# aliftffd/ViT-vs-Raw-IQ

Hardware: AMD Instinct MI355X
Metric: IQ frames/sec training (fwd+loss+bwd+clip+AdamW) (higher is better)
Workload: dtype bf16; 1 GPU; ViT-Tiny/16 224x224 C=1 19cls (BASELINE configs[1]); config_id=B, per_gpu_batch=256, global_batch=256, parallelism=dp1, hipgraph=True

## Files before the change

### include/iqvit.h

```cpp
#ifndef IQVIT_H
#define IQVIT_H
#include <stddef.h>
#include <stdint.h>

#ifdef __cplusplus
extern "C" {
#endif

typedef void* iq_stream_t;

enum { IQ_STATUS_OK = 0, IQ_STATUS_ARG = 1, IQ_STATUS_UNSUPPORTED = 2, IQ_STATUS_LAUNCH = 3 };

typedef struct iq_dropout {
  uint64_t seed;
  uint32_t step;
  uint32_t site;
  float p;
  const uint32_t* step_dev;
} iq_dropout_t;
#define IQ_SITE_IMPAIR 0xFFFFFFFFu
#define IQ_SITE_SYNTH 0xFFFFFFFEu

int iq_ln_supported(int D);
int iq_ln_fwd(const void* z, const float* gamma, const float* beta, void* x, float* mean, float* rstd, int M, int D,
              float eps, iq_stream_t stream);
size_t iq_ln_bwd_ws_bytes(int D);
int iq_ln_bwd(const void* dx, const void* z, const float* mean, const float* rstd, const float* gamma, void* dz,
              void* dy, const iq_dropout_t* drop, float* dgamma, float* dbeta, float* ws, int accumulate, int M,
              int D, iq_stream_t stream);
int iq_ln_bwd_partial_rows(int M, int D);

typedef struct iq_epilogue {
  const float* bias;
  int relu;
  const float* pe;
  int tok, seq, cls_off;
  iq_dropout_t drop;
  const void* gate;
  int ldg;
  float gate_scale;
  const void* residual;
  int ldr;
} iq_epilogue_t;
int iq_gemm_bf16_nt(const void* A, int lda, const void* B, int ldb, void* C, int ldc, int M, int N, int K,
                    const iq_epilogue_t* epi, iq_stream_t stream);

int iq_gemm_ln_supported(int D, int K);
int iq_gemm_bf16_ln(const void* A, int lda, const void* W, int ldw, const float* bias, const void* residual, int ldr,
                    const iq_dropout_t* drop, const float* gamma, const float* beta, float eps, void* Z, void* X,
                    float* mean, float* rstd, int M, int D, int K, iq_stream_t stream);
// ... 25 lines not shown
                              const iq_dropout_t* drop2, const float* gamma2, const float* beta2, float eps, void* Z2, void* X,
                              float* mean2, float* rstd2, void* gate_bits, const void* Wq, const float* bq, void* Yq, int frames,
                              int S, int D, int F, iq_stream_t stream);

size_t iq_wgrad_ws_bytes(int M, int N, int K);
int iq_gemm_bf16_wgrad(const void* dY, int ldy, const void* X, int ldx, float* dW, float* dbias, int M, int N, int K,
                       float* ws, size_t ws_bytes, int accumulate, iq_stream_t stream);

typedef struct iq_wgrad_problem {
  const void* dY;
  int ldy;
  const void* X;
  int ldx;
  float* dW;
  float* dbias;
  int N, K;
} iq_wgrad_problem_t;
typedef struct iq_reduce_seg {
  const float* partials;
  int rows;
  int64_t row_stride;
  float* out;
  int64_t n;
} iq_reduce_seg_t;
size_t iq_wgrad_grouped_ws_bytes(const iq_wgrad_problem_t* probs, int nprob, int M, int max_workgroups);
int iq_gemm_bf16_wgrad_grouped(const iq_wgrad_problem_t* probs, int nprob, int M, float* ws, size_t ws_bytes,
                               int accumulate, int max_workgroups, const iq_reduce_seg_t* extra, int nextra,
                               iq_stream_t stream);

int iq_attn_supported(int S, int dh);
int iq_attn_fwd(const void* qkv, void* out, float* lse, int B, int S, int H, int dh, iq_stream_t stream);
int iq_attn_bwd(const void* qkv, const void* out, const void* dout, const float* lse, void* dqkv, int B, int S, int H,
                int dh, iq_stream_t stream);
int iq_attn_fwd_masked(const void* qkv, void* out, float* lse, const uint8_t* mask, long mask_hstride, int B, int S,
                       int H, int dh, iq_stream_t stream);
int iq_attn_bwd_masked(const void* qkv, const void* out, const void* dout, const float* lse, void* dqkv,
                       const uint8_t* mask, long mask_hstride, int B, int S, int H, int dh, iq_stream_t stream);
int iq_attn_probs(const void* qkv, const float* lse, float* out, long out_bstride, int B, int S, int H, int dh,
                  int rows, int heads, iq_stream_t stream);
int iq_attn_grad_probs(const void* qkv, const float* lse, const void* dout, float* out, long out_bstride, int B, int S,
                       int H, int dh, int rows, int heads, int positive, iq_stream_t stream);
int iq_attn_relevance_step(const void* qkv, const float* lse, const void* dout, const float* r_in, float* r_out, int B,
                           int S, int H, int dh, iq_stream_t stream);

int iq_frames_preprocess(const float* raw, float* out, int n_frames, int len, int take, const float* stats,
                         iq_stream_t stream);
typedef struct iq_impair {
  float phase_lo, phase_hi;
  float cfo_lo, cfo_hi;
  int   rot90;
  int   conj;
  int   shift_max;
  float gain_db_lo, gain_db_hi;
  float snr_db_lo, snr_db_hi;
  uint64_t seed; uint32_t step;
  uint64_t frame_base;
} iq_impair_t;
int iq_frames_impair(const float* raw, float* out, float* drawn, int n_frames, int len, int take, const float* stats,
                     const iq_impair_t* imp, iq_stream_t stream);
#define IQ_SYNTH_MAX_CLASSES 128
#define IQ_SYNTH_MAX_SNRS 64
typedef struct iq_synth_class { int kind; int offset; int count; } iq_synth_class_t;
typedef struct iq_synth {
  const float* points;
  const iq_synth_class_t* classes; int n_classes;
  const float* snrs_db; int n_snrs;
// ... 26 lines not shown
size_t iq_gradnorm_ws_bytes(size_t n);
int iq_gradnorm_sq(const float* g, size_t n, float grad_scale, float* ws, float* out, iq_stream_t stream);
int iq_adamw_step(float* p, const float* g, float* m, float* v, void* shadow_bf16, size_t n, float lr, float beta1,
                  float beta2, float eps, float weight_decay, int step, const float* gnorm_sq, float max_norm,
                  float grad_scale, const float* dyn, iq_stream_t stream);
int iq_counter_add(uint32_t* ctr_u32, uint32_t inc_u32, float* ctr_f32, float inc_f32, iq_stream_t stream);
int iq_cast_bf16(const float* src, void* dst, size_t n, iq_stream_t stream);
int iq_transpose_cast_bf16(const float* src, void* dst, int rows, int cols, iq_stream_t stream);

typedef struct iq_model_cfg {
  int kind;
  int in_channels;
  int img_h, img_w, patch;
  int seq_length, conv_k, use_cls;
  int num_classes, d_model, n_head, n_layers, ffn_hidden;
  float drop_prob;
} iq_model_cfg_t;

typedef struct iq_model iq_model_t;

int iq_model_create(const iq_model_cfg_t* cfg, iq_model_t** out);
void iq_model_destroy(iq_model_t* m);
const char* iq_model_last_error(const iq_model_t* m);
int iq_model_tokens(const iq_model_t* m);
size_t iq_model_param_floats(const iq_model_t* m);
int iq_model_param_entries(const iq_model_t* m);
int iq_model_param_entry(const iq_model_t* m, int i, char* name, int name_cap, size_t* offset, int* ndim, int* dims);
size_t iq_model_shadow_bytes(const iq_model_t* m);
size_t iq_model_workspace_bytes(const iq_model_t* m, int batch, int training);
int iq_model_bind(iq_model_t* m, float* params, float* grads, const float* pe, void* shadow);
int iq_model_bind_step_counter(iq_model_t* m, uint32_t* counter);
int iq_model_refresh_shadow(iq_model_t* m, iq_stream_t stream);
int iq_model_refresh_transposed(iq_model_t* m, iq_stream_t stream);
int iq_model_forward(iq_model_t* m, const float* src, int batch, void* workspace, size_t ws_bytes, int training,
                     uint64_t seed, uint32_t step, float* enc_out, float* logits, iq_stream_t stream);
int iq_model_backward(iq_model_t* m, const float* dlogits, const float* denc, int batch, void* workspace,
                      size_t ws_bytes, int accumulate, int stage_hi, int stage_lo, iq_stream_t stream);
int iq_model_grad_range(const iq_model_t* m, int stage_hi, int stage_lo, size_t* off, size_t* len);
#define IQ_BWD_PARAM_GRADS 1
int iq_model_backward_input(iq_model_t* m, const float* dlogits, const float* denc, int batch, void* workspace,
                            size_t ws_bytes, float* dsrc, int flags, iq_stream_t stream);
int iq_model_attention(iq_model_t* m, const void* workspace, size_t ws_bytes, int batch, int layer, int rows,
                       int heads, float* out, long out_bstride, iq_stream_t stream);
int iq_model_attention_rollout(iq_model_t* m, const void* workspace, size_t ws_bytes, int batch, float alpha,
                               float* out, iq_stream_t stream);
int iq_model_attention_relevance(iq_model_t* m, const float* dlogits, int batch, void* workspace, size_t ws_bytes,
                                 float* rel, float* const* maps, int rows, int heads, int positive, long out_bstride,
                                 iq_stream_t stream);

#define IQ_PROF_FAMILIES 8
int iq_prof_enable(int on);
int iq_prof_collect(double* ms, long long* count);
size_t iq_prof_kernels(char* out, size_t cap, int reset);

#ifdef __cplusplus
}
#endif
#endif
```

### vit-vs-raw-iq_amd/_native.py

```python
from __future__ import annotations

import ctypes as C
import os

_HERE = os.path.dirname(os.path.abspath(__file__))
LIB_PATH = os.environ.get("IQ_LIBIQVIT") or os.path.join(_HERE, "libiqvit.so")

BWD_PARAM_GRADS = 1

STATUS = {0: "ok", 1: "invalid argument", 2: "unsupported shape/configuration", 3: "HIP launch error"}


class IqError(RuntimeError):
    pass


class Dropout(C.Structure):
    _fields_ = [("seed", C.c_uint64), ("step", C.c_uint32), ("site", C.c_uint32), ("p", C.c_float),
                ("step_dev", C.c_void_p)]


class Impair(C.Structure):
    _fields_ = [("phase_lo", C.c_float), ("phase_hi", C.c_float), ("cfo_lo", C.c_float), ("cfo_hi", C.c_float),
                ("rot90", C.c_int), ("conj", C.c_int), ("shift_max", C.c_int), ("gain_db_lo", C.c_float),
                ("gain_db_hi", C.c_float), ("snr_db_lo", C.c_float), ("snr_db_hi", C.c_float), ("seed", C.c_uint64),
                ("step", C.c_uint32), ("frame_base", C.c_uint64)]


class SynthClass(C.Structure):
    _fields_ = [("kind", C.c_int), ("offset", C.c_int), ("count", C.c_int)]


class Synth(C.Structure):
    _fields_ = [("points", C.c_void_p), ("classes", C.POINTER(SynthClass)), ("n_classes", C.c_int),
                ("snrs_db", C.POINTER(C.c_float)), ("n_snrs", C.c_int), ("balanced", C.c_int), ("seed", C.c_uint64),
                ("stream", C.c_uint32), ("frame_base", C.c_uint64)]


class Epilogue(C.Structure):
    _fields_ = [("bias", C.c_void_p), ("relu", C.c_int), ("pe", C.c_void_p), ("tok", C.c_int), ("seq", C.c_int),
                ("cls_off", C.c_int), ("drop", Dropout), ("gate", C.c_void_p), ("ldg", C.c_int),
                ("gate_scale", C.c_float), ("residual", C.c_void_p), ("ldr", C.c_int)]


class WgradProblem(C.Structure):
    _fields_ = [("dY", C.c_void_p), ("ldy", C.c_int), ("X", C.c_void_p), ("ldx", C.c_int), ("dW", C.c_void_p),
                ("dbias", C.c_void_p), ("N", C.c_int), ("K", C.c_int)]


class ReduceSeg(C.Structure):
    _fields_ = [("partials", C.c_void_p), ("rows", C.c_int), ("row_stride", C.c_int64), ("out", C.c_void_p),
                ("n", C.c_int64)]
# ... 9 lines not shown
_P, _I, _Z, _F = C.c_void_p, C.c_int, C.c_size_t, C.c_float
_U64, _U32 = C.c_uint64, C.c_uint32

SIGNATURES = {
    "iq_ln_supported": (_I, [_I]),
    "iq_ln_fwd": (_I, [_P, _P, _P, _P, _P, _P, _I, _I, _F, _P]),
    "iq_ln_bwd_ws_bytes": (_Z, [_I]),
    "iq_ln_bwd_partial_rows": (_I, [_I, _I]),
    "iq_ln_bwd": (_I, [_P, _P, _P, _P, _P, _P, _P, C.POINTER(Dropout), _P, _P, _P, _I, _I, _I, _P]),
    "iq_gemm_bf16_nt": (_I, [_P, _I, _P, _I, _P, _I, _I, _I, _I, C.POINTER(Epilogue), _P]),
    "iq_gemm_ln_supported": (_I, [_I, _I]),
    "iq_gemm_bf16_ln": (_I, [_P, _I, _P, _I, _P, _P, _I, C.POINTER(Dropout), _P, _P, _F, _P, _P, _P, _P, _I, _I, _I, _P]),
    "iq_gemm_lnbwd_supported": (_I, [_I, _I]),
    "iq_gemm_lnbwd_partial_rows": (_I, [_I]),
    "iq_gemm_bf16_lnbwd": (_I, [_P, _I, _P, _I, _P, _I, _P, _P, _P, _P, C.POINTER(Dropout), _P, _P, _P, _I, _I, _I, _P]),
    "iq_ffn_chain_supported": (_I, [_I, _I, _I]),
    "iq_ffn_chain_bwd_partial_rows": (_I, [_I]),
    "iq_ffn_chain_bwd": (_I, [_P, _P, _P, _F, _P, _P, _P, _P, _P, _P, _P, C.POINTER(Dropout), _P, _P, _P, _P, _P, _I, _I, _I, _I, _P]),
    "iq_qkv_dgrad_ffn_chain_bwd": (_I, [_P, _P, _P, _P, _P, _P, _P, C.POINTER(Dropout), _P, _P, _P,
                                        _P, _P, _F, _P, _P, _P, _P, _P, _P, _P, C.POINTER(Dropout), _P, _P, _P, _P, _P, _I, _I, _I, _I, _P]),
    "iq_ffn_chain_gate_bytes": (_Z, [_I, _I]),
    "iq_ffn_chain_fwd": (_I, [_P, _P, _P, C.POINTER(Dropout), _P, _P, _P, C.POINTER(Dropout), _P, _P, _F, _P, _P, _P, _P, _P, _I, _I,
                              _I, _I, _P]),
    "iq_attn_out_ffn_chain_fwd": (_I, [_P, _P, _P, C.POINTER(Dropout), _P, _P, _P, _P, _P, _P, _P,
                                       _P, _P, C.POINTER(Dropout), _P, _P, _P, C.POINTER(Dropout), _P, _P, _F, _P, _P, _P, _P, _P,
                                       _P, _P, _P, _I, _I, _I, _I, _P]),
    "iq_wgrad_ws_bytes": (_Z, [_I, _I, _I]),
    "iq_gemm_bf16_wgrad": (_I, [_P, _I, _P, _I, _P, _P, _I, _I, _I, _P, _Z, _I, _P]),
    "iq_wgrad_grouped_ws_bytes": (_Z, [_P, _I, _I, _I]),
    "iq_gemm_bf16_wgrad_grouped": (_I, [_P, _I, _I, _P, _Z, _I, _I, _P, _I, _P]),
    "iq_attn_supported": (_I, [_I, _I]),
    "iq_attn_fwd": (_I, [_P, _P, _P, _I, _I, _I, _I, _P]),
    "iq_attn_bwd": (_I, [_P, _P, _P, _P, _P, _I, _I, _I, _I, _P]),
    "iq_attn_fwd_masked": (_I, [_P, _P, _P, _P, C.c_long, _I, _I, _I, _I, _P]),
    "iq_attn_bwd_masked": (_I, [_P, _P, _P, _P, _P, _P, C.c_long, _I, _I, _I, _I, _P]),
    "iq_attn_probs": (_I, [_P, _P, _P, C.c_long, _I, _I, _I, _I, _I, _I, _P]),
    "iq_attn_grad_probs": (_I, [_P, _P, _P, _P, C.c_long, _I, _I, _I, _I, _I, _I, _I, _P]),
    "iq_attn_relevance_step": (_I, [_P, _P, _P, _P, _P, _I, _I, _I, _I, _P]),
    "iq_frames_preprocess": (_I, [_P, _P, _I, _I, _I, C.POINTER(C.c_float), _P]),
    "iq_frames_impair": (_I, [_P, _P, _P, _I, _I, _I, C.POINTER(C.c_float), C.POINTER(Impair), _P]),
    "iq_frames_synth": (_I, [_P, _P, _P, _P, _P, _I, _I, C.POINTER(Synth), _P]),
    "iq_patchify": (_I, [_P, _P, _I, _I, _I, _I, _I, _I, _I, _P]),
    "iq_cls_rows": (_I, [_P, _P, _P, _I, _I, _I, C.POINTER(Dropout), _P]),
    "iq_embed_bwd_gather": (_I, [_P, _P, _P, _I, _I, _I, _I, _I, C.POINTER(Dropout), _I, _P]),
    "iq_embed_dgrad": (_I, [_P, _P, _I, _P, _I, _I, _I, _I, _I, _I, _I, _P]),
    "iq_linf_step": (_I, [_P, _P, _P, _F, _F, _F, _F, _Z, _P]),
    "iq_head_fwd": (_I, [_P, _P, _P, _P, _P, _P, _P, _P, _I, _I, _I, _I, _I, _P]),
    "iq_ce_fwd_bwd": (_I, [_P, _P, _I, _I, _F, _F, _P, _P, _P, _P]),
    "iq_head_bwd": (_I, [_P, _P, _P, _P, _P, _P, _P, _P, _P, _P, _P, _I, _I, _I, _I, _I, _I, _P]),
    "iq_gradnorm_ws_bytes": (_Z, [_Z]),
    "iq_gradnorm_sq": (_I, [_P, _Z, _F, _P, _P, _P]),
    "iq_adamw_step": (_I, [_P, _P, _P, _P, _P, _Z, _F, _F, _F, _F, _F, _I, _P, _F, _F, _P, _P]),
    "iq_counter_add": (_I, [_P, _U32, _P, _F, _P]),
    "iq_cast_bf16": (_I, [_P, _P, _Z, _P]),
    "iq_transpose_cast_bf16": (_I, [_P, _P, _I, _I, _P]),
    "iq_model_create": (_I, [C.POINTER(ModelCfg), C.POINTER(_P)]),
    "iq_model_destroy": (None, [_P]),
    "iq_model_last_error": (C.c_char_p, [_P]),
    "iq_model_tokens": (_I, [_P]),
    "iq_model_param_floats": (_Z, [_P]),
    "iq_model_param_entries": (_I, [_P]),
    "iq_model_param_entry": (_I, [_P, _I, C.c_char_p, _I, C.POINTER(_Z), C.POINTER(_I), C.POINTER(_I)]),
    "iq_model_shadow_bytes": (_Z, [_P]),
    "iq_model_workspace_bytes": (_Z, [_P, _I, _I]),
    "iq_model_bind": (_I, [_P, _P, _P, _P, _P]),
    "iq_model_bind_step_counter": (_I, [_P, _P]),
# ... 52 lines not shown
```

### vit-vs-raw-iq_amd/csrc/attention.hip

```cpp
#include <stdlib.h>

#include "common.h"
#include "iqvit.h"
#include "prof.h"

namespace {

constexpr int ATT_THREADS = 512;
constexpr int ATT_WAVES = ATT_THREADS / 64;
constexpr float LOG2E = 1.4426950408889634f;
constexpr float LN2 = 0.6931471805599453f;
constexpr float NEG_BIG = -1.0e30f;

__device__ __forceinline__ float fast_exp2(float x) { return __builtin_amdgcn_exp2f(x); }

template <int DH> struct AttCfg {
  static constexpr int LD = (DH == 16) ? 16 : DH + 16;
  static constexpr int KS = (DH + 31) / 32;
  static constexpr int DT = DH / 16;
  static constexpr int CPR = DH / 8;
};

typedef __attribute__((address_space(3))) s16x4 lds_s16x4;

// ... 50 lines not shown
#pragma unroll
    for (int j = 0; j < UN; ++j) {
      const int id = base + j * ATT_THREADS + tid;
      const int r = id / CPR, c = id % CPR;
      if (id < total) {
        const bool live = r_begin + r < S;
        *reinterpret_cast<bf16x8*>(imgA + r * LD + c * 8) = live ? va[j] : bf16x8{};
        *reinterpret_cast<bf16x8*>(imgB + r * LD + c * 8) = live ? vb[j] : bf16x8{};
      }
    }
  }
}

__device__ __forceinline__ bf16x8 pack_b(const f32x4& lo, const f32x4& hi) {
  bf16x8 v;
#pragma unroll
  for (int r = 0; r < 4; ++r) { v[r] = (bf16)lo[r]; v[4 + r] = (bf16)hi[r]; }
  return v;
}

__device__ __forceinline__ float group4_max(float v) {
  v = fmaxf(v, __shfl_xor(v, 16, 64));
  return fmaxf(v, __shfl_xor(v, 32, 64));
}
__device__ __forceinline__ float group4_sum(float v) {
  v += __shfl_xor(v, 16, 64);
  return v + __shfl_xor(v, 32, 64);
}

template <int DH, bool MASKED>
__global__ __launch_bounds__(ATT_THREADS) void attn_fwd_kernel(const bf16* __restrict__ qkv, bf16* __restrict__ out,
                                                               float* __restrict__ lse, const uint8_t* __restrict__ mask,
                                                               long mask_hstride, int S, int H, int kchunk,
                                                               float scale_log2, float masked_raw) {
  using C = AttCfg<DH>;
  extern __shared__ __attribute__((aligned(16))) unsigned char smem[];
  bf16* Ks = reinterpret_cast<bf16*>(smem);
  bf16* Vs = Ks + kchunk * C::LD;
  const int tid = threadIdx.x, lane = tid & 63, wave = tid >> 6, g = lane >> 4, c16 = lane & 15;
  const int b = blockIdx.x / H, h = blockIdx.x % H;
  const int D = H * DH;
  const long ldg = 3L * D;
  const bf16* qb = qkv + (long)b * S * ldg + h * DH;
  const bf16* kb_ = qb + D;
  const bf16* vb_ = qb + 2 * D;
  const uint8_t* mk = MASKED ? mask + (long)b * (mask_hstride ? (long)H * S * S : (long)S * S) + h * mask_hstride : nullptr;
  const int qtiles = (S + 31) / 32, npass = (qtiles + ATT_WAVES - 1) / ATT_WAVES, nstage = (S + kchunk - 1) / kchunk;

  if (nstage == 1) {
    stage_pair<DH, 4>(Ks, kb_, ldg, Vs, vb_, ldg, 0, min(kchunk, ((S + 31) / 32) * 32), S, tid);
    __syncthreads();
  }
  for (int pass = 0; pass < npass; ++pass) {
    const int qt = pass * ATT_WAVES + wave;
    const bool active = qt < qtiles;
    bf16x8 qf[2][C::KS];
    f32x4 o[2][C::DT];
    float m[2], lsum[2];
#pragma unroll
    for (int u = 0; u < 2; ++u) {
      m[u] = NEG_BIG; lsum[u] = 0.f;
#pragma unroll
      for (int s = 0; s < C::KS; ++s) qf[u][s] = row_frag_gmem<DH>(qb, ldg, qt * 32 + u * 16 + c16, active ? S : 0, s, lane);
#pragma unroll
      for (int dt = 0; dt < C::DT; ++dt) o[u][dt] = f32x4{0.f, 0.f, 0.f, 0.f};
    }
    for (int st = 0; st < nstage; ++st) {
      const int k0 = st * kchunk;
      const int krows = min(kchunk, ((S - k0 + 31) / 32) * 32);
      if (nstage > 1) {
        __syncthreads();
        stage_pair<DH, 2>(Ks, kb_, ldg, Vs, vb_, ldg, k0, krows, S, tid);
        __syncthreads();
      }
      if (active) {
        const bool u1 = qt * 32 + 16 < S;
        for (int kb = 0; kb < krows; kb += 32) {
          const bool k1 = k0 + kb + 16 < S;
          const bool kpad = k0 + kb + 32 > S;
          f32x4 sc[2][2];
// ... 65 lines not shown
            const bf16x8 vt = tr_frag(Vs, C::LD, kb, dt * 16, lane);
            o[0][dt] = __builtin_amdgcn_mfma_f32_16x16x32_bf16(vt, pb[0], o[0][dt], 0, 0, 0);
            if (u1) o[1][dt] = __builtin_amdgcn_mfma_f32_16x16x32_bf16(vt, pb[1], o[1][dt], 0, 0, 0);
          }
        }
      }
    }
    if (active) {
#pragma unroll
      for (int u = 0; u < 2; ++u) {
        const float l = group4_sum(lsum[u]);
        const float inv = 1.0f / l;
        const int q = qt * 32 + u * 16 + c16;
        if (q < S) {
#pragma unroll
          for (int dt = 0; dt < C::DT; ++dt) {
            bf16x4 w;
#pragma unroll
            for (int r = 0; r < 4; ++r) w[r] = (bf16)(o[u][dt][r] * inv);
            *reinterpret_cast<bf16x4*>(out + ((long)b * S + q) * D + h * DH + dt * 16 + 4 * g) = w;
          }
          if (g == 0) lse[((long)b * H + h) * S + q] = (m[u] + log2f(l)) * LN2;
        }
      }
    }
  }
}

template <int DH, bool MASKED>
__global__ __launch_bounds__(ATT_THREADS, 4) void attn_bwd_kernel(const bf16* __restrict__ qkv, const bf16* __restrict__ out,
                                                               const bf16* __restrict__ dout, const float* __restrict__ lse,
                                                               bf16* __restrict__ dqkv, const uint8_t* __restrict__ mask,
                                                               long mask_hstride, int S, int H, int spad, int chunk,
                                                               float scale, float masked_raw) {
  using C = AttCfg<DH>;
  extern __shared__ __attribute__((aligned(16))) unsigned char smem[];
  bf16* I0 = reinterpret_cast<bf16*>(smem);
  bf16* I1 = I0 + chunk * C::LD;
  float* lse_s = reinterpret_cast<float*>(I1 + chunk * C::LD);
  float* del_s = lse_s + spad;
  const int tid = threadIdx.x, lane = tid & 63, wave = tid >> 6, g = lane >> 4, c16 = lane & 15;
  const int b = blockIdx.x / H, h = blockIdx.x % H;
  const int D = H * DH;
  const long ldg = 3L * D;
  const bf16* qb = qkv + (long)b * S * ldg + h * DH;
  const bf16* kb_ = qb + D;
  const bf16* vb_ = qb + 2 * D;
  const bf16* ob = out + (long)b * S * D + h * DH;
  const bf16* dob = dout + (long)b * S * D + h * DH;
  bf16* dqb = dqkv + (long)b * S * ldg + h * DH;
  const uint8_t* mk = MASKED ? mask + (long)b * (mask_hstride ? (long)H * S * S : (long)S * S) + h * mask_hstride : nullptr;
  const float scale_log2 = scale * LOG2E;
  const int nblk = spad / 32;
  const int nchunk = (spad + chunk - 1) / chunk;
  const bool single = nchunk == 1;

  if (single) {
    stage_pair<DH, 4>(I0, qb, ldg, I1, dob, (long)D, 0, spad, S, tid);
    __syncthreads();
  }
  for (int q = tid; q < spad; q += ATT_THREADS) {
    float dl = 0.f, ls = 0.f;
    if (q < S) {
#pragma unroll
      for (int c = 0; c < C::CPR; ++c) {
        const bf16x8 a = single ? *reinterpret_cast<const bf16x8*>(I1 + q * C::LD + c * 8)
                                : *reinterpret_cast<const bf16x8*>(dob + (long)q * D + c * 8);
        const bf16x8 o8 = *reinterpret_cast<const bf16x8*>(ob + (long)q * D + c * 8);
#pragma unroll
        for (int e = 0; e < 8; ++e) dl += (float)a[e] * (float)o8[e];
      }
      ls = lse[((long)b * H + h) * S + q] * LOG2E;
    }
    del_s[q] = dl;
    lse_s[q] = ls;
  }
  __syncthreads();

  const int nunit = (S + 15) / 16;
  for (int ug = 0; ug * ATT_WAVES < nunit; ++ug) {
    const int unit = ug * ATT_WAVES + wave;
    const bool have = unit < nunit;
    bf16x8 kf[C::KS], vf[C::KS];
#pragma unroll
    for (int s = 0; s < C::KS; ++s) {
      kf[s] = row_frag_gmem<DH>(kb_, ldg, unit * 16 + c16, have ? S : 0, s, lane);
      vf[s] = row_frag_gmem<DH>(vb_, ldg, unit * 16 + c16, have ? S : 0, s, lane);
    }
    f32x4 dv[C::DT], dk[C::DT];
#pragma unroll
    for (int dt = 0; dt < C::DT; ++dt) { dv[dt] = f32x4{0.f, 0.f, 0.f, 0.f}; dk[dt] = f32x4{0.f, 0.f, 0.f, 0.f}; }
    const int key = unit * 16 + c16;
    const bool unit_partial = unit * 16 + 16 > S;
    for (int qc = 0; qc < nchunk; ++qc) {
      const int q0 = qc * chunk;
      const int rows = min(chunk, spad - q0);
      if (!single) {
        __syncthreads();
        stage_pair<DH, 2>(I0, qb, ldg, I1, dob, (long)D, q0, rows, S, tid);
        __syncthreads();
      }
      if (!have) continue;
      for (int ql = 0; ql < rows; ql += 32) {
        const bool u1 = q0 + ql + 16 < S;
        f32x4 p[2], ds[2];
#pragma unroll
        for (int u = 0; u < 2; ++u) {
          if (u == 1 && !u1) { p[1] = f32x4{0.f, 0.f, 0.f, 0.f}; ds[1] = f32x4{0.f, 0.f, 0.f, 0.f}; continue; }
          f32x4 sa = {0.f, 0.f, 0.f, 0.f}, dp = {0.f, 0.f, 0.f, 0.f};
#pragma unroll
          for (int s = 0; s < C::KS; ++s) {
            const bf16x8 qa = row_frag_lds<DH>(I0, ql + u * 16 + c16, s, lane);
            const bf16x8 da = row_frag_lds<DH>(I1, ql + u * 16 + c16, s, lane);
            sa = __builtin_amdgcn_mfma_f32_16x16x32_bf16(qa, kf[s], sa, 0, 0, 0);
            dp = __builtin_amdgcn_mfma_f32_16x16x32_bf16(da, vf[s], dp, 0, 0, 0);
          }
#pragma unroll
          for (int r = 0; r < 4; ++r) {
            const int q = q0 + ql + u * 16 + 4 * g + r;
            bool blocked = false;
            if (MASKED) blocked = q < S && key < S && !mk[(long)q * S + key];
            float pv = fast_exp2((blocked ? masked_raw : sa[r]) * scale_log2 - lse_s[q]);
            if (unit_partial) pv = key < S ? pv : 0.f;
            p[u][r] = pv;
            ds[u][r] = blocked ? 0.f : pv * (dp[r] - del_s[q]) * scale;
          }
        }
        const bf16x8 pB = pack_b(p[0], p[1]), dsB = pack_b(ds[0], ds[1]);
#pragma unroll
        for (int dt = 0; dt < C::DT; ++dt) {
          const bf16x8 doT = tr_frag(I1, C::LD, ql, dt * 16, lane);
          const bf16x8 qT = tr_frag(I0, C::LD, ql, dt * 16, lane);
// ... 6 lines not shown
#pragma unroll
      for (int dt = 0; dt < C::DT; ++dt) {
        bf16x4 wk, wv;
#pragma unroll
        for (int r = 0; r < 4; ++r) { wk[r] = (bf16)dk[dt][r]; wv[r] = (bf16)dv[dt][r]; }
        *reinterpret_cast<bf16x4*>(dqb + (long)key * ldg + D + dt * 16 + 4 * g) = wk;
        *reinterpret_cast<bf16x4*>(dqb + (long)key * ldg + 2 * D + dt * 16 + 4 * g) = wv;
      }
    }
  }

  bf16x8 qf[2][C::KS], dof[2][C::KS];
  if (single) {
#pragma unroll
    for (int u = 0; u < 2; ++u)
#pragma unroll
      for (int s = 0; s < C::KS; ++s) {
        const int q = min(wave, nblk - 1) * 32 + u * 16 + c16;
        qf[u][s] = row_frag_lds<DH>(I0, q, s, lane);
        dof[u][s] = row_frag_lds<DH>(I1, q, s, lane);
      }
  }
  for (int qg = 0; qg * ATT_WAVES < nblk; ++qg) {
    const int qblk = qg * ATT_WAVES + wave;
    const bool have = qblk < nblk;
    float lq[2], dl[2];
#pragma unroll
    for (int u = 0; u < 2; ++u) {
      const int q = min(qblk, nblk - 1) * 32 + u * 16 + c16;
      if (!single || qg != 0) {
#pragma unroll
        for (int s = 0; s < C::KS; ++s) {
          qf[u][s] = row_frag_gmem<DH>(qb, ldg, q, have ? S : 0, s, lane);
          dof[u][s] = row_frag_gmem<DH>(dob, (long)D, q, have ? S : 0, s, lane);
        }
      }
      lq[u] = lse_s[q];
      dl[u] = del_s[q];
    }
    f32x4 dq[C::DT][2];
#pragma unroll
    for (int dt = 0; dt < C::DT; ++dt)
#pragma unroll
      for (int u = 0; u < 2; ++u) dq[dt][u] = f32x4{0.f, 0.f, 0.f, 0.f};
    for (int kc = 0; kc < nchunk; ++kc) {
      const int k0 = kc * chunk;
      const int rows = min(chunk, spad - k0);
      if (!single || qg == 0) {
        __syncthreads();
        stage_pair<DH, 2>(I0, kb_, ldg, I1, vb_, ldg, k0, rows, S, tid);
        __syncthreads();
      }
      if (!have) continue;
      const bool u1 = qblk * 32 + 16 < S;
      for (int kl = 0; kl < rows; kl += 32) {
        const bool kblk_partial = k0 + kl + 32 > S;
        const bool k1 = k0 + kl + 16 < S;
        f32x4 ds[2][2];
#pragma unroll
        for (int kt = 0; kt < 2; ++kt) {
          if (kt == 1 && !k1) { ds[0][1] = f32x4{0.f, 0.f, 0.f, 0.f}; ds[1][1] = f32x4{0.f, 0.f, 0.f, 0.f}; continue; }
          bf16x8 ka[C::KS], va[C::KS];
#pragma unroll
          for (int s = 0; s < C::KS; ++s) {
            ka[s] = row_frag_lds<DH>(I0, kl + kt * 16 + c16, s, lane);
            va[s] = row_frag_lds<DH>(I1, kl + kt * 16 + c16, s, lane);
          }
// ... 17 lines not shown
              float pv = fast_exp2((blocked ? masked_raw : sa[r]) * scale_log2 - lq[u]);
              if (kblk_partial) pv = key < S ? pv : 0.f;
              ds[u][kt][r] = blocked ? 0.f : pv * (dp[r] - dl[u]) * scale;
            }
          }
        }
        bf16x8 dsB[2];
#pragma unroll
        for (int u = 0; u < 2; ++u) dsB[u] = pack_b(ds[u][0], ds[u][1]);
#pragma unroll
        for (int dt = 0; dt < C::DT; ++dt) {
          const bf16x8 kT = tr_frag(I0, C::LD, kl, dt * 16, lane);
          dq[dt][0] = __builtin_amdgcn_mfma_f32_16x16x32_bf16(kT, dsB[0], dq[dt][0], 0, 0, 0);
          if (u1) dq[dt][1] = __builtin_amdgcn_mfma_f32_16x16x32_bf16(kT, dsB[1], dq[dt][1], 0, 0, 0);
        }
      }
    }
    if (have) {
#pragma unroll
      for (int u = 0; u < 2; ++u) {
        const int q = qblk * 32 + u * 16 + c16;
        if (q < S) {
#pragma unroll
          for (int dt = 0; dt < C::DT; ++dt) {
            bf16x4 w;
#pragma unroll
            for (int r = 0; r < 4; ++r) w[r] = (bf16)dq[dt][u][r];
            *reinterpret_cast<bf16x4*>(dqb + (long)q * ldg + dt * 16 + 4 * g) = w;
          }
        }
      }
    }
  }
}

constexpr int ONCE_MAX_SPAD = 224;
constexpr int ONCE_LD = 64;

__device__ __forceinline__ int once_off(int row, int col) { return row * ONCE_LD + (col ^ (((row >> 1) & 3) << 4)); }

__device__ __forceinline__ bf16x8 once_tr_frag(const bf16* tile, int r0, int dt, int lane) {
  const int i16 = lane & 15, g = lane >> 4;
  const bf16* a = tile + once_off(r0 + 4 * g + (i16 >> 2), dt * 16 + 4 * (i16 & 3));
  s16x4 lo = __builtin_amdgcn_ds_read_tr16_b64_v4i16((lds_s16x4*)(a));
  s16x4 hi = __builtin_amdgcn_ds_read_tr16_b64_v4i16((lds_s16x4*)(a + 16 * ONCE_LD));
  s16x8 v = {lo[0], lo[1], lo[2], lo[3], hi[0], hi[1], hi[2], hi[3]};
  return __builtin_bit_cast(bf16x8, v);
}
__device__ __forceinline__ bf16x8 once_row_frag(const bf16* tile, int row, int s, int lane) {
  return *reinterpret_cast<const bf16x8*>(tile + once_off(row, s * 32 + 8 * (lane >> 4)));
}

template <int NT, int UN, int NIMG>
__device__ __forceinline__ void once_stage(bf16* const (&img)[NIMG], const bf16* const (&base)[NIMG],
                                           const long (&ldg)[NIMG], int spad, int S, int tid) {
  const int total = spad * 8;
  for (int b0 = 0; b0 < total; b0 += UN * NT) {
    bf16x8 v[NIMG][UN];
#pragma unroll
    for (int j = 0; j < UN; ++j) {
      const int id = min(b0 + j * NT + tid, total - 1);
      const int r = min(id >> 3, S - 1), c = id & 7;
#pragma unroll
      for (int i = 0; i < NIMG; ++i) v[i][j] = *reinterpret_cast<const bf16x8*>(base[i] + (long)r * ldg[i] + c * 8);
    }
#pragma unroll
    for (int j = 0; j < UN; ++j) {
      const int id = b0 + j * NT + tid;
      const int r = id >> 3, c = id & 7;
      if (id < total) {
        const bool live = r < S;
#pragma unroll
        for (int i = 0; i < NIMG; ++i) *reinterpret_cast<bf16x8*>(img[i] + once_off(r, c * 8)) = live ? v[i][j] : bf16x8{};
      }
    }
  }
}

template <int NT>
__global__ __launch_bounds__(NT, 4) void attn_bwd_once_kernel(const bf16* __restrict__ qkv, const bf16* __restrict__ out,
                                                              const bf16* __restrict__ dout, const float* __restrict__ lse,
                                                              bf16* __restrict__ dqkv, int S, int H, int spad, float scale) {
  constexpr int DH = 64, KS = 2, DT = 4, NW = NT / 64;
  extern __shared__ __attribute__((aligned(16))) unsigned char smem[];
  bf16* I0 = reinterpret_cast<bf16*>(smem);
  bf16* I1 = I0 + spad * ONCE_LD;
  float* lse_s = reinterpret_cast<float*>(I1 + spad * ONCE_LD);
  float* del_s = lse_s + spad;
  bf16* dSi = reinterpret_cast<bf16*>(del_s + spad);
  const int tid = threadIdx.x, lane = tid & 63, wave = tid >> 6, g = lane >> 4, c16 = lane & 15;
  const int b = blockIdx.x / H, h = blockIdx.x % H;
  const int D = H * DH;
  const long ldg = 3L * D;
  const bf16* qb = qkv + (long)b * S * ldg + h * DH;
  const bf16* kb_ = qb + D;
  const bf16* vb_ = qb + 2 * D;
  const bf16* ob = out + (long)b * S * D + h * DH;
  const bf16* dob = dout + (long)b * S * D + h * DH;
  bf16* dqb = dqkv + (long)b * S * ldg + h * DH;
  const float scale_log2 = scale * LOG2E;
  const int nunit = (S + 15) / 16;
  const int ldS = nunit * 16 + 8;

  {
    bf16* const img[2] = {I0, I1};
    const bf16* const src[2] = {qb, dob};
    const long lds_[2] = {ldg, (long)D};
    once_stage<NT, 2048 / NT, 2>(img, src, lds_, spad, S, tid);
  }
  __syncthreads();
  for (int q = tid; q < spad; q += NT) {
    float dl = 0.f, ls = 0.f;
    if (q < S) {
#pragma unroll
      for (int c = 0; c < 8; ++c) {
        const bf16x8 a = *reinterpret_cast<const bf16x8*>(I1 + once_off(q, c * 8));
        const bf16x8 o8 = *reinterpret_cast<const bf16x8*>(ob + (long)q * D + c * 8);
#pragma unroll
        for (int e = 0; e < 8; ++e) dl += (float)a[e] * (float)o8[e];
      }
      ls = lse[((long)b * H + h) * S + q] * LOG2E;
    }
    del_s[q] = dl;
    lse_s[q] = ls;
  }
  __syncthreads();

  for (int unit = wave; unit < nunit; unit += NW) {
    bf16x8 kf[KS], vf[KS];
#pragma unroll
    for (int s = 0; s < KS; ++s) {
      kf[s] = row_frag_gmem<DH>(kb_, ldg, unit * 16 + c16, S, s, lane);
      vf[s] = row_frag_gmem<DH>(vb_, ldg, unit * 16 + c16, S, s, lane);
    }
    f32x4 dv[DT], dk[DT];
#pragma unroll
    for (int dt = 0; dt < DT; ++dt) { dv[dt] = f32x4{0.f, 0.f, 0.f, 0.f}; dk[dt] = f32x4{0.f, 0.f, 0.f, 0.f}; }
    const int key = unit * 16 + c16;
    const bool unit_partial = unit * 16 + 16 > S;
    for (int ql = 0; ql < spad; ql += 32) {
      const bool u1 = ql + 16 < S;
      f32x4 p[2], ds[2];
#pragma unroll
      for (int u = 0; u < 2; ++u) {
        if (u == 1 && !u1) { p[1] = f32x4{0.f, 0.f, 0.f, 0.f}; ds[1] = f32x4{0.f, 0.f, 0.f, 0.f}; continue; }
        f32x4 sa = {0.f, 0.f, 0.f, 0.f}, dp = {0.f, 0.f, 0.f, 0.f};
#pragma unroll
        for (int s = 0; s < KS; ++s) {
          const bf16x8 qa = once_row_frag(I0, ql + u * 16 + c16, s, lane);
          const bf16x8 da = once_row_frag(I1, ql + u * 16 + c16, s, lane);
          sa = __builtin_amdgcn_mfma_f32_16x16x32_bf16(qa, kf[s], sa, 0, 0, 0);
          dp = __builtin_amdgcn_mfma_f32_16x16x32_bf16(da, vf[s], dp, 0, 0, 0);
        }
        const f32x4 lq4 = *reinterpret_cast<const f32x4*>(lse_s + ql + u * 16 + 4 * g);
        const f32x4 dl4 = *reinterpret_cast<const f32x4*>(del_s + ql + u * 16 + 4 * g);
#pragma unroll
        for (int r = 0; r < 4; ++r) {
          float pv = fast_exp2(sa[r] * scale_log2 - lq4[r]);
          if (unit_partial) pv = key < S ? pv : 0.f;
          p[u][r] = pv;
          ds[u][r] = pv * (dp[r] - dl4[r]) * scale;
        }
      }
      const bf16x8 pB = pack_b(p[0], p[1]), dsB = pack_b(ds[0], ds[1]);
      bf16* w = dSi + (ql + 4 * g) * ldS + key;
#pragma unroll
      for (int r = 0; r < 4; ++r) w[r * ldS] = dsB[r];
      if (u1) {
#pragma unroll
        for (int r = 0; r < 4; ++r) w[(16 + r) * ldS] = dsB[4 + r];
      }
#pragma unroll
      for (int dt = 0; dt < DT; ++dt) {
        const bf16x8 doT = once_tr_frag(I1, ql, dt, lane);
        const bf16x8 qT = once_tr_frag(I0, ql, dt, lane);
        dv[dt] = __builtin_amdgcn_mfma_f32_16x16x32_bf16(doT, pB, dv[dt], 0, 0, 0);
        dk[dt] = __builtin_amdgcn_mfma_f32_16x16x32_bf16(qT, dsB, dk[dt], 0, 0, 0);
      }
    }
    if (key < S) {
#pragma unroll
      for (int dt = 0; dt < DT; ++dt) {
        bf16x4 wk, wv;
#pragma unroll
        for (int r = 0; r < 4; ++r) { wk[r] = (bf16)dk[dt][r]; wv[r] = (bf16)dv[dt][r]; }
        *reinterpret_cast<bf16x4*>(dqb + (long)key * ldg + D + dt * 16 + 4 * g) = wk;
        *reinterpret_cast<bf16x4*>(dqb + (long)key * ldg + 2 * D + dt * 16 + 4 * g) = wv;
      }
    }
  }

  __syncthreads();
  {
    bf16* const img[1] = {I0};
    const bf16* const src[1] = {kb_};
    const long lds_[1] = {ldg};
    once_stage<NT, 2048 / NT, 1>(img, src, lds_, spad, S, tid);
  }
  __syncthreads();
  for (int half = wave; half < nunit; half += NW) {
    const int q = half * 16 + c16;
    const bf16* drow = dSi + q * ldS + 4 * g;
    f32x4 dq[DT];
#pragma unroll
    for (int dt = 0; dt < DT; ++dt) dq[dt] = f32x4{0.f, 0.f, 0.f, 0.f};
    for (int kl = 0; kl < spad; kl += 32) {
      const bool k1 = kl + 16 < S;
      const bf16x4 lo = *reinterpret_cast<const bf16x4*>(drow + kl);
      bf16x4 hi = {};
      if (k1) hi = *reinterpret_cast<const bf16x4*>(drow + kl + 16);
      const bf16x8 dsB = {lo[0], lo[1], lo[2], lo[3], hi[0], hi[1], hi[2], hi[3]};
#pragma unroll
      for (int dt = 0; dt < DT; ++dt) {
        const bf16x8 kT = once_tr_frag(I0, kl, dt, lane);
        dq[dt] = __builtin_amdgcn_mfma_f32_16x16x32_bf16(kT, dsB, dq[dt], 0, 0, 0);
      }
    }
    if (q < S) {
#pragma unroll
      for (int dt = 0; dt < DT; ++dt) {
        bf16x4 w;
#pragma unroll
        for (int r = 0; r < 4; ++r) w[r] = (bf16)dq[dt][r];
        *reinterpret_cast<bf16x4*>(dqb + (long)q * ldg + dt * 16 + 4 * g) = w;
      }
    }
  }
}

template <int DH>
__device__ __forceinline__ bf16x8 row_frag_img(const bf16* tile, int ld, int row, int s, int lane) {
  const int d0 = s * 32 + 8 * (lane >> 4);
  bf16x8 v = {};
  if (DH >= 32 || d0 < DH) v = *reinterpret_cast<const bf16x8*>(tile + row * ld + d0);
// ... 376 lines not shown
  return iq_launch_status();
}
template <int DH>
int launch_frame_bwd(const void* qkv, const void* out, const void* dout, const float* lse, void* dqkv, int B, int S, int H,
                     hipStream_t st) {
  const int spad = (S + 31) / 32 * 32;
  const size_t lds = frame_bwd_lds(S, H, DH);
  auto k = attn_frame_bwd_kernel<DH, (DH == 64 ? 2 : 3), (DH == 16 ? 4 : DH == 32 ? 3 : 2)>;
  if (lds > 48 * 1024) (void)hipFuncSetAttribute((const void*)k, hipFuncAttributeMaxDynamicSharedMemorySize, (int)lds);
  const int threads = 64 * (H < ATT_WAVES ? H : ATT_WAVES);
  k<<<B, threads, lds, st>>>((const bf16*)qkv, (const bf16*)out, (const bf16*)dout, lse, (bf16*)dqkv, S, H, spad,
                             1.0f / sqrtf((float)DH));
  return iq_launch_status();
}

constexpr size_t ATT_LDS_FWD_BUDGET = 72 * 1024;
constexpr size_t ATT_LDS_BWD_BUDGET = 76 * 1024;
constexpr int ATT_MAX_S = 4096;

template <int DH> int bwd_chunk_rows(int S) {
  const int spad = (S + 31) / 32 * 32;
  const long room = (long)ATT_LDS_BWD_BUDGET - (long)2 * spad * sizeof(float);
  int chunk = (int)(room / (2 * AttCfg<DH>::LD * 2)) / 32 * 32;
  if (chunk > spad) chunk = spad;
  return chunk;
}
template <int DH> size_t bwd_lds_bytes(int S) {
  const int spad = (S + 31) / 32 * 32;
  return (size_t)2 * bwd_chunk_rows<DH>(S) * AttCfg<DH>::LD * 2 + (size_t)2 * spad * sizeof(float);
}

template <int DH, bool MASKED>
int launch_fwd(const void* qkv, void* out, float* lse, const uint8_t* mask, long mask_hstride, int B, int S, int H,
               hipStream_t st) {
  const int spad = (S + 31) / 32 * 32;
  int kchunk = (int)(ATT_LDS_FWD_BUDGET / (2 * AttCfg<DH>::LD * 2)) / 32 * 32;
  if (kchunk > spad) kchunk = spad;
  const size_t lds = (size_t)2 * kchunk * AttCfg<DH>::LD * 2;
  const float scale_log2 = LOG2E / sqrtf((float)DH);
  if (lds > 48 * 1024)
    (void)hipFuncSetAttribute((const void*)attn_fwd_kernel<DH, MASKED>, hipFuncAttributeMaxDynamicSharedMemorySize, (int)lds);
  attn_fwd_kernel<DH, MASKED><<<B * H, ATT_THREADS, lds, st>>>((const bf16*)qkv, (bf16*)out, lse, mask, mask_hstride, S, H,
                                                               kchunk, scale_log2, -10000.0f * sqrtf((float)DH));
  return iq_launch_status();
}

template <int DH, bool MASKED>
int launch_bwd(const void* qkv, const void* out, const void* dout, const float* lse, void* dqkv, const uint8_t* mask,
               long mask_hstride, int B, int S, int H, hipStream_t st) {
  const int spad = (S + 31) / 32 * 32;
  const int chunk = bwd_chunk_rows<DH>(S);
  if (S > ATT_MAX_S || chunk < 32) return IQ_ERR_UNSUPPORTED;
  const size_t lds = bwd_lds_bytes<DH>(S);
  if (lds > 48 * 1024)
    (void)hipFuncSetAttribute((const void*)attn_bwd_kernel<DH, MASKED>, hipFuncAttributeMaxDynamicSharedMemorySize, (int)lds);
  attn_bwd_kernel<DH, MASKED><<<B * H, ATT_THREADS, lds, st>>>((const bf16*)qkv, (const bf16*)out, (const bf16*)dout, lse,
                                                               (bf16*)dqkv, mask, mask_hstride, S, H, spad, chunk,
                                                               1.0f / sqrtf((float)DH), -10000.0f * sqrtf((float)DH));
  return iq_launch_status();
}

inline int once_threads(int S, int dh, bool masked) {
  static const int tune = [] { const char* e = getenv("IQ_TUNE_ATTN_BWD_ONCE"); return e ? atoi(e) : -1; }();
  if (masked || dh != 64 || (S + 31) / 32 * 32 > ONCE_MAX_SPAD || tune == 0) return 0;
  return tune == 512 ? 512 : 1024;
}
template <int NT>
int launch_bwd_once(const void* qkv, const void* out, const void* dout, const float* lse, void* dqkv, int B, int S, int H,
                    hipStream_t st) {
  const int spad = (S + 31) / 32 * 32, nunit = (S + 15) / 16;
  const size_t lds = (size_t)2 * spad * ONCE_LD * 2 + (size_t)2 * spad * sizeof(float) + (size_t)spad * (nunit * 16 + 8) * 2;
  auto k = attn_bwd_once_kernel<NT>;
  if (lds > 48 * 1024) (void)hipFuncSetAttribute((const void*)k, hipFuncAttributeMaxDynamicSharedMemorySize, (int)lds);
  k<<<B * H, NT, lds, st>>>((const bf16*)qkv, (const bf16*)out, (const bf16*)dout, lse, (bf16*)dqkv, S, H, spad,
                            1.0f / sqrtf(64.0f));
  return iq_launch_status();
}

template <bool MASKED>
int dispatch_fwd(const void* qkv, void* out, float* lse, const uint8_t* mask, long hs, int B, int S, int H, int dh,
                 hipStream_t st) {
  switch (dh) {
    case 16: return launch_fwd<16, MASKED>(qkv, out, lse, mask, hs, B, S, H, st);
    case 32: return launch_fwd<32, MASKED>(qkv, out, lse, mask, hs, B, S, H, st);
    case 64: return launch_fwd<64, MASKED>(qkv, out, lse, mask, hs, B, S, H, st);
    default: return IQ_ERR_UNSUPPORTED;
  }
}
template <bool MASKED>
int dispatch_bwd(const void* qkv, const void* out, const void* dout, const float* lse, void* dqkv, const uint8_t* mask,
                 long hs, int B, int S, int H, int dh, hipStream_t st) {
  switch (dh) {
    case 16: return launch_bwd<16, MASKED>(qkv, out, dout, lse, dqkv, mask, hs, B, S, H, st);
    case 32: return launch_bwd<32, MASKED>(qkv, out, dout, lse, dqkv, mask, hs, B, S, H, st);
    case 64: return launch_bwd<64, MASKED>(qkv, out, dout, lse, dqkv, mask, hs, B, S, H, st);
    default: return IQ_ERR_UNSUPPORTED;
  }
}

}

extern "C" int iq_attn_supported(int S, int dh) {
  if (S <= 0 || S > ATT_MAX_S) return 0;
  return (dh == 16 || dh == 32 || dh == 64) ? 1 : 0;
}

extern "C" int iq_attn_fwd_masked(const void* qkv, void* out, float* lse, const uint8_t* mask, long mask_hstride, int B,
                                  int S, int H, int dh, iq_stream_t stream) {
  if (B <= 0) return IQ_OK;
  if (!qkv || !out || !lse || S <= 0 || H <= 0) return IQ_ERR_ARG;
  if (mask_hstride != 0 && mask_hstride != (long)S * S) return IQ_ERR_ARG;
  hipStream_t st = (hipStream_t)stream;
  IQ_PROF(IQ_FAM_ATTN_FWD, st);
  const bool frame = !mask && (dh == 16 || dh == 32 || dh == 64) && use_frame(S, frame_fwd_lds(S, H, dh));
  {
    const double rows = (double)B * S, Dm = (double)H * dh;
    if (frame) IQ_PROF_K(2.0 * rows * 4.0 * Dm + 4.0 * B * H * S, 4.0 * B * H * (double)S * S * dh, "attn_frame_fwd_kernel<%d>", dh);
    else IQ_PROF_K(2.0 * rows * 4.0 * Dm + 4.0 * B * H * S, 4.0 * B * H * (double)S * S * dh, "attn_fwd_kernel<%d, %s>", dh, mask ? "true" : "false");
  }
  if (frame) {
    switch (dh) {
      case 16: return launch_frame_fwd<16>(qkv, out, lse, B, S, H, st);
      case 32: return launch_frame_fwd<32>(qkv, out, lse, B, S, H, st);
      default: return launch_frame_fwd<64>(qkv, out, lse, B, S, H, st);
    }
  }
  return mask ? dispatch_fwd<true>(qkv, out, lse, mask, mask_hstride, B, S, H, dh, st)
              : dispatch_fwd<false>(qkv, out, lse, nullptr, 0, B, S, H, dh, st);
}
extern "C" int iq_attn_fwd(const void* qkv, void* out, float* lse, int B, int S, int H, int dh, iq_stream_t stream) {
  return iq_attn_fwd_masked(qkv, out, lse, nullptr, 0, B, S, H, dh, stream);
}

extern "C" int iq_attn_bwd_masked(const void* qkv, const void* out, const void* dout, const float* lse, void* dqkv,
                                  const uint8_t* mask, long mask_hstride, int B, int S, int H, int dh,
                                  iq_stream_t stream) {
  if (B <= 0) return IQ_OK;
  if (!qkv || !out || !dout || !lse || !dqkv || S <= 0 || H <= 0) return IQ_ERR_ARG;
  if (mask_hstride != 0 && mask_hstride != (long)S * S) return IQ_ERR_ARG;
  hipStream_t st = (hipStream_t)stream;
  IQ_PROF(IQ_FAM_ATTN_BWD, st);
  const bool frame = !mask && (dh == 16 || dh == 32 || dh == 64) && use_frame(S, frame_bwd_lds(S, H, dh));
  const int once = frame ? 0 : once_threads(S, dh, mask != nullptr);
  {
    const double rows = (double)B * S, Dm = (double)H * dh;
    if (frame) IQ_PROF_K(2.0 * rows * 8.0 * Dm + 4.0 * B * H * S, 14.0 * B * H * (double)S * S * dh, "attn_frame_bwd_kernel<%d>", dh);
    else if (once) IQ_PROF_K(2.0 * rows * 8.0 * Dm + 4.0 * B * H * S, 10.0 * B * H * (double)S * S * dh, "attn_bwd_once_kernel<%d>", once);
    else IQ_PROF_K(2.0 * rows * 8.0 * Dm + 4.0 * B * H * S, 14.0 * B * H * (double)S * S * dh, "attn_bwd_kernel<%d, %s>", dh, mask ? "true" : "false");
  }
  if (frame) {
    switch (dh) {
      case 16: return launch_frame_bwd<16>(qkv, out, dout, lse, dqkv, B, S, H, st);
      case 32: return launch_frame_bwd<32>(qkv, out, dout, lse, dqkv, B, S, H, st);
      default: return launch_frame_bwd<64>(qkv, out, dout, lse, dqkv, B, S, H, st);
    }
  }
  if (once == 512) return launch_bwd_once<512>(qkv, out, dout, lse, dqkv, B, S, H, st);
  if (once) return launch_bwd_once<1024>(qkv, out, dout, lse, dqkv, B, S, H, st);
  return mask ? dispatch_bwd<true>(qkv, out, dout, lse, dqkv, mask, mask_hstride, B, S, H, dh, st)
              : dispatch_bwd<false>(qkv, out, dout, lse, dqkv, nullptr, 0, B, S, H, dh, st);
}
extern "C" int iq_attn_bwd(const void* qkv, const void* out, const void* dout, const float* lse, void* dqkv, int B,
                           int S, int H, int dh, iq_stream_t stream) {
  return iq_attn_bwd_masked(qkv, out, dout, lse, dqkv, nullptr, 0, B, S, H, dh, stream);
}
```

### vit-vs-raw-iq_amd/csrc/common.h

```cpp
#pragma once
#include <hip/hip_runtime.h>
#include <stdint.h>

#include "../../include/iqvit.h"

typedef __bf16 bf16;
typedef __attribute__((ext_vector_type(8))) __bf16 bf16x8;
typedef __attribute__((ext_vector_type(4))) __bf16 bf16x4;
typedef __attribute__((ext_vector_type(4))) short s16x4;
typedef __attribute__((ext_vector_type(8))) short s16x8;
typedef __attribute__((ext_vector_type(4))) float f32x4;
typedef __attribute__((ext_vector_type(4))) uint32_t u32x4;
typedef __attribute__((address_space(3))) void lds_void_t;
typedef __attribute__((address_space(1))) const void gbl_cvoid_t;

#define IQ_OK 0
#define IQ_ERR_ARG 1
#define IQ_ERR_UNSUPPORTED 2
#define IQ_ERR_LAUNCH 3

#define IQ_WAVE 64

static inline int iq_launch_status() {
  hipError_t e = hipGetLastError();
  return e == hipSuccess ? IQ_OK : IQ_ERR_LAUNCH;
}

__device__ __forceinline__ float bf2f(bf16 v) { return (float)v; }
__device__ __forceinline__ bf16 f2bf(float v) { return (bf16)v; }

__device__ __forceinline__ void unpack8(const bf16x8& v, float* f) {
#pragma unroll
  for (int i = 0; i < 8; ++i) f[i] = (float)v[i];
}
__device__ __forceinline__ bf16x8 pack8(const float* f) {
  bf16x8 v;
#pragma unroll
  for (int i = 0; i < 8; ++i) v[i] = (bf16)f[i];
  return v;
}

struct IqRng {
  uint64_t seed;
  uint32_t step;
  uint32_t site;
  const uint32_t* step_dev;
};

__device__ __forceinline__ IqRng rng_resolve(IqRng r) {
  if (r.step_dev) r.step = *r.step_dev;
  return r;
}

#ifndef IQ_PHILOX_ROUNDS
#define IQ_PHILOX_ROUNDS 7
#endif
__device__ __forceinline__ u32x4 philox4x32(uint32_t c0, uint32_t c1, uint32_t c2, uint32_t c3,
                                            uint32_t k0, uint32_t k1) {
  const uint32_t M0 = 0xD2511F53u, M1 = 0xCD9E8D57u, W0 = 0x9E3779B9u, W1 = 0xBB67AE85u;
#pragma unroll
  for (int r = 0; r < IQ_PHILOX_ROUNDS; ++r) {
    const uint64_t p0 = (uint64_t)M0 * (uint64_t)c0;
    const uint64_t p1 = (uint64_t)M1 * (uint64_t)c2;
    const uint32_t n0 = (uint32_t)(p1 >> 32) ^ c1 ^ k0, n1 = (uint32_t)p1;
    const uint32_t n2 = (uint32_t)(p0 >> 32) ^ c3 ^ k1, n3 = (uint32_t)p0;
    c0 = n0; c1 = n1; c2 = n2; c3 = n3;
    k0 += W0; k1 += W1;
  }
  u32x4 o = {c0, c1, c2, c3};
  return o;
}

__device__ __forceinline__ float u24(uint32_t w) { return (float)(w >> 8) * 0x1p-24f; }
__device__ __forceinline__ float u24_open(uint32_t w) { return (float)((w >> 8) + 1u) * 0x1p-24f; }
__device__ __forceinline__ void box_muller(uint32_t a, uint32_t b, float& g0, float& g1) {
  const float r = sqrtf(-2.f * logf(u24_open(a)));
  float sn, cs;
  sincospif(2.f * u24(b), &sn, &cs);
  g0 = r * cs;
  g1 = r * sn;
}

__device__ __forceinline__ uint32_t dropout_keep8(const IqRng& r, uint64_t group, uint32_t thresh) {
  u32x4 b = philox4x32((uint32_t)group, (uint32_t)(group >> 32), r.site, r.step,
                          (uint32_t)r.seed, (uint32_t)(r.seed >> 32));
  uint32_t m = 0;
#pragma unroll
  for (int i = 0; i < 4; ++i) {
    m |= ((b[i] & 0xFFFFu) >= thresh ? 1u : 0u) << (2 * i);
    m |= ((b[i] >> 16) >= thresh ? 1u : 0u) << (2 * i + 1);
  }
  return m;
}

__host__ __device__ inline uint32_t dropout_thresh(float p) {
  float t = p * 65536.0f + 0.5f;
  if (t < 0.f) t = 0.f;
  if (t > 65535.f) t = 65535.f;
  return (uint32_t)t;
}
__host__ __device__ inline float dropout_scale(float p) {
  uint32_t t = dropout_thresh(p);
  return 65536.0f / (65536.0f - (float)t);
}

inline bool dropout_unpack(const iq_dropout_t* d, int* on, IqRng* rng, uint32_t* thresh, float* dscale) {
  *on = 0; *rng = IqRng{0, 0, 0, nullptr}; *thresh = 0; *dscale = 1.f;
  if (!d || !(d->p > 0.f)) return true;
  *on = 1;
  *rng = IqRng{d->seed, d->step, d->site, d->step_dev};
  *thresh = dropout_thresh(d->p);
  *dscale = dropout_scale(d->p);
  return d->p < 1.f;
}

constexpr int vmcnt_imm(int n) { return (n & 15) | ((n >> 4) << 14) | 0x0F70; }

__device__ __forceinline__ int xcd_remap(int bid, int nwg) {
  const int NX = 8;
  int q = nwg / NX, r = nwg % NX;
  int xcd = bid % NX, idx = bid / NX;
  int base = (xcd < r) ? xcd * (q + 1) : r * (q + 1) + (xcd - r) * q;
  return base + idx;
}

__device__ __forceinline__ float wave_sum(float v) {
#pragma unroll
  for (int o = 32; o > 0; o >>= 1) v += __shfl_xor(v, o, 64);
  return v;
}
__device__ __forceinline__ float wave_max(float v) {
#pragma unroll
  for (int o = 32; o > 0; o >>= 1) v = fmaxf(v, __shfl_xor(v, o, 64));
  return v;
}
```

### vit-vs-raw-iq_amd/csrc/ffn_chain.hip

```cpp
#include <stdlib.h>

#include <type_traits>

#include "common.h"
#include "iqvit.h"
#include "prof.h"

namespace {

constexpr int FC_CHUNK = 64, FC_NS = 3, FC_MAXW = 7;

struct FfnChainParams {
  const bf16* X1; const bf16* W1; const bf16* W2;
  const float* b1; const float* b2; const float* gamma; const float* beta;
  bf16* H; bf16* Z; bf16* X; float* mean; float* rstd;
  uint32_t* gate;
  int M, F;
  float eps;
  int drop1_on, drop2_on; IqRng rng1, rng2; uint32_t thresh1, thresh2; float dscale1, dscale2;
  const bf16* A0; const bf16* W0; const bf16* R0; const float* b0; const float* gamma0; const float* beta0;
  bf16* Z0; bf16* X1out; float* mean0; float* rstd0;
  int drop0_on; IqRng rng0; uint32_t thresh0; float dscale0;
  const bf16* Wq; const float* bq; bf16* Yq;
};
// ... 1030 lines not shown
  return sh.nw == 5 ? launch_chain_bwd<D, 5, 1>(p, st) : launch_chain_bwd<D, 8, 1>(p, st);
}

}

extern "C" int iq_ffn_chain_supported(int S, int D, int F) {
  if (!(D == 128 || D == 192) || F < FC_CHUNK || (F % FC_CHUNK) || S <= 0) return 0;
  return (size_t)FC_NS * 2 * FC_CHUNK * D * 2 + ((size_t)F + 9 * D) * sizeof(float) <= (size_t)160 * 1024 ? 1 : 0;
}

namespace {
struct ChainPre {
  const void* A0; const void* W0; const float* b0; const iq_dropout_t* drop0; const void* R0;
  const float* gamma0; const float* beta0; void* Z0; float* mean0; float* rstd0;
  const void* Wq; const float* bq; void* Yq;
};

int chain_fwd(const ChainPre* pre, const void* X1, const void* W1, const float* b1, const iq_dropout_t* drop1, void* H, const void* W2,
              const float* b2, const iq_dropout_t* drop2, const float* gamma, const float* beta, float eps, void* Z, void* X,
              float* mean, float* rstd, void* gate_bits, int frames, int S, int D, int F, iq_stream_t stream) {
  if (frames <= 0) return IQ_OK;
  if (!X1 || !W1 || !b1 || !H || !W2 || !b2 || !gamma || !beta || !Z || !X || !mean || !rstd) return IQ_ERR_ARG;
  if (!iq_ffn_chain_supported(S, D, F)) return IQ_ERR_UNSUPPORTED;
  if (((uintptr_t)X1 | (uintptr_t)W1 | (uintptr_t)W2 | (uintptr_t)H | (uintptr_t)Z | (uintptr_t)X | (uintptr_t)b1 | (uintptr_t)b2 |
       (uintptr_t)gamma | (uintptr_t)beta) % 16) return IQ_ERR_ARG;
  if ((long)frames * S > 0x7FFFFFFFL) return IQ_ERR_UNSUPPORTED;
  FfnChainParams p = {};
  p.X1 = (const bf16*)X1; p.W1 = (const bf16*)W1; p.W2 = (const bf16*)W2;
  p.b1 = b1; p.b2 = b2; p.gamma = gamma; p.beta = beta;
  p.H = (bf16*)H; p.Z = (bf16*)Z; p.X = (bf16*)X; p.mean = mean; p.rstd = rstd;
  p.gate = (uint32_t*)gate_bits;
  if ((uintptr_t)gate_bits % 16) return IQ_ERR_ARG;
  p.M = frames * S; p.F = F; p.eps = eps;
  if (!dropout_unpack(drop1, &p.drop1_on, &p.rng1, &p.thresh1, &p.dscale1) ||
      !dropout_unpack(drop2, &p.drop2_on, &p.rng2, &p.thresh2, &p.dscale2)) return IQ_ERR_ARG;
  if (pre) {
    if (!pre->A0 || !pre->W0 || !pre->b0 || !pre->R0 || !pre->gamma0 || !pre->beta0 || !pre->Z0 || !pre->mean0 || !pre->rstd0)
      return IQ_ERR_ARG;
    if (((uintptr_t)pre->A0 | (uintptr_t)pre->W0 | (uintptr_t)pre->b0 | (uintptr_t)pre->R0 | (uintptr_t)pre->gamma0 |
         (uintptr_t)pre->beta0 | (uintptr_t)pre->Z0) % 16) return IQ_ERR_ARG;
    p.A0 = (const bf16*)pre->A0; p.W0 = (const bf16*)pre->W0; p.R0 = (const bf16*)pre->R0; p.b0 = pre->b0;
    p.gamma0 = pre->gamma0; p.beta0 = pre->beta0; p.Z0 = (bf16*)pre->Z0; p.X1out = (bf16*)X1; p.mean0 = pre->mean0; p.rstd0 = pre->rstd0;
    if (!dropout_unpack(pre->drop0, &p.drop0_on, &p.rng0, &p.thresh0, &p.dscale0)) return IQ_ERR_ARG;
    if (pre->Wq || pre->bq || pre->Yq) {
      if (!pre->Wq || !pre->bq || !pre->Yq || ((uintptr_t)pre->Wq | (uintptr_t)pre->bq | (uintptr_t)pre->Yq) % 16) return IQ_ERR_ARG;
      p.Wq = (const bf16*)pre->Wq; p.bq = pre->bq; p.Yq = (bf16*)pre->Yq;
    }
  }
  hipStream_t st = (hipStream_t)stream;
  IQ_PROF(IQ_FAM_GEMM_NT, st);
  const double M = (double)p.M;
  double more_bytes = 0.0, more_flops = 0.0;
  if (pre) { more_bytes += 2.0 * (M * D * 3 + (double)D * D) + 8.0 * M; more_flops += 2.0 * M * D * D; }
  if (p.Wq) { more_bytes += 2.0 * (M * 3 * D + 3.0 * D * D); more_flops += 6.0 * M * D * D; }
  IQ_PROF_K(2.0 * (M * D * 3 + M * F + 2.0 * D * F) + 8.0 * M + more_bytes, 4.0 * M * D * F + more_flops,
            "ffn_chain_fwd_kernel<%d, %d, %d, %s, %d>", D, chain_waves(p.M), chain_shape(p.M).rg, p.drop1_on ? "true" : "false", p.Wq ? 2 : pre ? 1 : 0);
  return D == 192 ? launch_chain_d<192>(p, st) : launch_chain_d<128>(p, st);
}
}

extern "C" int iq_ffn_chain_fwd(const void* X1, const void* W1, const float* b1, const iq_dropout_t* drop1, void* H,
                                const void* W2, const float* b2, const iq_dropout_t* drop2, const float* gamma,
                                const float* beta, float eps, void* Z, void* X, float* mean, float* rstd, void* gate_bits,
                                int frames, int S, int D, int F, iq_stream_t stream) {
  return chain_fwd(nullptr, X1, W1, b1, drop1, H, W2, b2, drop2, gamma, beta, eps, Z, X, mean, rstd, gate_bits, frames, S, D, F, stream);
}
// ... 12 lines not shown
  if (M <= 0) return 0;
  const int nw = chain_waves(M);
  return (int)((chain_units(M) + nw - 1) / nw);
}

extern "C" size_t iq_ffn_chain_gate_bytes(int M, int F) {
  if (M <= 0 || F <= 0) return 0;
  return (size_t)chain_units(M) * (size_t)(F / FC_CHUNK) * 64 * sizeof(uint32_t);
}

namespace {
struct ChainBwdPre {
  const void* A0; const void* W0t; const void* R0; const void* Z0; const float* mean0; const float* rstd0; const float* gamma0;
  const iq_dropout_t* drop0; void* dZ0; void* dY0; float* partial0;
};

int chain_bwd(const ChainBwdPre* pre, const void* dO, const void* W2t, const void* gate_bits, float gate_scale, void* gH, const void* W1t,
              const void* residual, const void* z1, const float* mean, const float* rstd, const float* gamma, const iq_dropout_t* drop,
              void* dz, void* dy, float* partial, const void* Wot, void* dA, int frames, int S, int D, int F, iq_stream_t stream) {
  if (frames <= 0) return IQ_OK;
  if ((Wot == nullptr) != (dA == nullptr) || ((uintptr_t)Wot | (uintptr_t)dA) % 16) return IQ_ERR_ARG;
  if ((!pre && !dO) || !W2t || !gate_bits || !gH || !W1t || !residual || !z1 || !mean || !rstd || !gamma || !dz || !partial) return IQ_ERR_ARG;
  if (!iq_ffn_chain_supported(S, D, F)) return IQ_ERR_UNSUPPORTED;
  if (((uintptr_t)dO | (uintptr_t)W2t | (uintptr_t)W1t | (uintptr_t)gate_bits | (uintptr_t)gH | (uintptr_t)residual | (uintptr_t)z1 |
       (uintptr_t)dz | (uintptr_t)dy | (uintptr_t)gamma | (uintptr_t)partial) % 16) return IQ_ERR_ARG;
  if ((long)frames * S > 0x7FFFFFFFL) return IQ_ERR_UNSUPPORTED;
  FfnChainBwdParams p = {};
  p.dO = (const bf16*)dO; p.W2t = (const bf16*)W2t; p.W1t = (const bf16*)W1t;
  p.gate = (const uint32_t*)gate_bits; p.R = (const bf16*)residual; p.Z1 = (const bf16*)z1;
  p.mean = mean; p.rstd = rstd; p.gamma = gamma;
  p.gH = (bf16*)gH; p.dZ = (bf16*)dz; p.dY = (bf16*)dy; p.partial = partial;
  p.M = frames * S; p.F = F; p.gate_scale = gate_scale;
  p.Wot = (const bf16*)Wot; p.dA = (bf16*)dA;
  if (!dropout_unpack(drop, &p.drop_on, &p.rng, &p.thresh, &p.dscale) || (p.drop_on && !dy)) return IQ_ERR_ARG;
  if (pre) {
    if (!Wot) return IQ_ERR_ARG;
    if (!pre->A0 || !pre->W0t || !pre->R0 || !pre->Z0 || !pre->mean0 || !pre->rstd0 || !pre->gamma0 || !pre->dZ0 || !pre->partial0)
      return IQ_ERR_ARG;
    if (((uintptr_t)pre->A0 | (uintptr_t)pre->W0t | (uintptr_t)pre->R0 | (uintptr_t)pre->Z0 | (uintptr_t)pre->gamma0 |
         (uintptr_t)pre->dZ0 | (uintptr_t)pre->dY0 | (uintptr_t)pre->partial0) % 16) return IQ_ERR_ARG;
    const float p0 = pre->drop0 ? pre->drop0->p : 0.f, p1 = drop ? drop->p : 0.f;
    if (p0 != p1 || (p.drop_on && !pre->dY0)) return IQ_ERR_ARG;
    p.A0 = (const bf16*)pre->A0; p.W0t = (const bf16*)pre->W0t; p.R0 = (const bf16*)pre->R0; p.Z0 = (const bf16*)pre->Z0;
    p.mean0 = pre->mean0; p.rstd0 = pre->rstd0; p.gamma0 = pre->gamma0;
    p.dZ0 = (bf16*)pre->dZ0; p.dY0 = (bf16*)pre->dY0; p.partial0 = pre->partial0;
    int on0; uint32_t thresh0; float dscale0;
    (void)dropout_unpack(pre->drop0, &on0, &p.rng0, &thresh0, &dscale0);
  }
  hipStream_t st = (hipStream_t)stream;
  IQ_PROF(IQ_FAM_GEMM_NT, st);
  const double M = (double)p.M;
  double bytes = 2.0 * (M * D * (4 + (p.drop_on ? 1 : 0) + (Wot ? 1 : 0)) + 2.0 * M * F + 2.0 * D * F + (Wot ? (double)D * D : 0.0)) + 8.0 * M;
  double flops = 4.0 * M * D * F + (Wot ? 2.0 * M * D * D : 0.0);
  if (pre) {
    bytes += 2.0 * (M * 3 * D + M * D * (3 + (p.drop_on ? 1 : 0) - 1) + 3.0 * D * D) + 8.0 * M;
    flops += 6.0 * M * D * D;
  }
  IQ_PROF_K(bytes, flops, "ffn_chain_bwd_kernel<%d, %d, %d, %s, %d>", D, chain_waves(p.M), chain_shape(p.M).rg, p.drop_on ? "true" : "false", pre ? 2 : Wot ? 1 : 0);
  return D == 192 ? launch_chain_bwd_d<192>(p, st) : launch_chain_bwd_d<128>(p, st);
}
}

extern "C" int iq_ffn_chain_bwd(const void* dO, const void* W2t, const void* gate_bits, float gate_scale, void* gH, const void* W1t,
                                const void* residual, const void* z1, const float* mean, const float* rstd, const float* gamma,
                                const iq_dropout_t* drop, void* dz, void* dy, float* partial, const void* Wot, void* dA, int frames,
                                int S, int D, int F, iq_stream_t stream) {
// ... 15 lines not shown
```

### vit-vs-raw-iq_amd/csrc/gemm_common.h

```cpp
#pragma once
#include "common.h"

struct GemmParams {
#ifdef IQ_GEMM_STAMPS
  unsigned long long* stamps;
#endif
  const bf16* A; const bf16* B; bf16* C;
  int lda, ldb, ldc, M, N, K;
  const float* bias; int relu;
  const float* pe; int tok, seq, cls_off;
  int drop_on; IqRng rng; uint32_t thresh; float dscale;
  const bf16* gate; int ldg; float gate_scale;
  const bf16* residual; int ldr;
  int tiles_m, tiles_n;
  int stagger;
};

constexpr int EPI_RES = 1, EPI_GATE = 2, EPI_PE = 4;

template <int MT, int NT, int EPI>
struct EpiRegs {
  static constexpr int NP = NT / 2;
  f32x4 bias_lo[NP], bias_hi[NP];
  bf16x8 res[(EPI & EPI_RES) ? MT : 1][NP], gt[(EPI & EPI_GATE) ? MT : 1][NP];
// ... 76 lines not shown
#pragma unroll
  for (int i = 0; i < MT; ++i) {
    const int gm = row0 + i * 16 + c16;
    long orow = gm;
    int prow = 0;
    if (EPI & EPI_PE) {
      const int f = gm / p.tok, tk = gm - f * p.tok;
      prow = tk + p.cls_off;
      orow = (long)f * p.seq + prow;
    }
#pragma unroll
    for (int jp = 0; jp < NP; ++jp) {
      float w[8];
#pragma unroll
      for (int r = 0; r < 4; ++r) {
        const float va = acc[i][2 * jp][r], vb = acc[i][2 * jp + 1][r];
        const auto sw = __builtin_amdgcn_permlane16_swap(__float_as_uint(va), __float_as_uint(vb), false, false);
        w[r] = __uint_as_float(sw[0]) + R.bias_lo[jp][r];
        w[4 + r] = __uint_as_float(sw[1]) + R.bias_hi[jp][r];
      }
      const int col = col0 + (odd ? (2 * jp + 1) * 16 + 4 * (g - 1) : (2 * jp) * 16 + 4 * g);
      if (gm < p.M && col < p.N) {
        if (p.relu) {
#pragma unroll
          for (int e = 0; e < 8; ++e) w[e] = fmaxf(w[e], 0.f);
        }
        if (EPI & EPI_PE) {
          const f32x4 pa = *reinterpret_cast<const f32x4*>(p.pe + (long)prow * p.N + col);
          const f32x4 pb = *reinterpret_cast<const f32x4*>(p.pe + (long)prow * p.N + col + 4);
#pragma unroll
          for (int e = 0; e < 4; ++e) { w[e] += pa[e]; w[4 + e] += pb[e]; }
        }
        if (p.drop_on) {
          const uint32_t keep = dropout_keep8(rng, (uint64_t)(orow * p.N + col) >> 3, p.thresh);
#pragma unroll
          for (int e = 0; e < 8; ++e) w[e] = ((keep >> e) & 1u) ? w[e] * p.dscale : 0.f;
        }
        if (EPI & EPI_GATE) {
#pragma unroll
          for (int e = 0; e < 8; ++e) w[e] = ((float)R.gt[i][jp][e] > 0.f) ? w[e] * p.gate_scale : 0.f;
        }
        if (EPI & EPI_RES) {
#pragma unroll
          for (int e = 0; e < 8; ++e) w[e] += (float)R.res[i][jp][e];
        }
        const bf16x8 packed = pack8(w);
        if (LDSOUT) {
          const int lr = lrow0 + i * 16 + c16, lc = (lcol0 + (col - col0)) >> 3;
          *reinterpret_cast<bf16x8*>(hs + lr * 256 + ((lc ^ (lr & 15)) << 4)) = packed;
        }
#ifdef IQ_EPI_NO_STORE
        if (p.ldc < 0)
#endif
        *reinterpret_cast<bf16x8*>(p.C + orow * p.ldc + col) = packed;
      }
    }
  }
}

template <int MT, int NT, int EPI, bool LDSOUT = false>
__device__ __forceinline__ void gemm_epilogue(const GemmParams& p, f32x4 (&acc)[MT][NT], int row0, int col0, int lane,
                                              unsigned char* hs = nullptr, int lrow0 = 0, int lcol0 = 0) {
  EpiRegs<MT, NT, EPI> R;
  epi_load<MT, NT, EPI>(p, R, row0, col0, lane);
  __builtin_amdgcn_s_waitcnt(0x0F70);
  epi_finish<MT, NT, EPI, LDSOUT>(p, acc, R, row0, col0, lane, hs, lrow0, lcol0);
}
// ... 3 lines not shown
```

### vit-vs-raw-iq_amd/csrc/gemm_ln.hip

```cpp
#include <stdlib.h>

#include "common.h"
#include "gemm_common.h"
#include "gemm_ring.h"
#include "iqvit.h"
#include "prof.h"

namespace {

constexpr int LNG_THREADS = 256;

struct GemmLnParams {
  const bf16* A; const bf16* B;
  bf16* Z; bf16* X;
  int lda, ldb, M, K;
  const float* bias;
  int drop_on; IqRng rng; uint32_t thresh; float dscale;
  const bf16* residual; int ldr;
  const float* gamma; const float* beta;
  float* mean; float* rstd;
  float eps;
};

template <int BMT, int BN>
// ... 88 lines not shown
#pragma unroll
      for (int j = 0; j < NT; ++j)
        acc[i][j] = __builtin_amdgcn_mfma_f32_16x16x32_bf16(bfr[j], af[i], acc[i][j], 0, 0, 0);
  };
  for (int ks = 0; ks + 2 < nk; ++ks) {
    wait_barrier<PER_STAGE>();
    issue(ks + 2);
    compute(ks);
  }
  wait_barrier<PER_STAGE>();
  issue_tail();
  asm volatile("" ::: "memory");
  compute(nk - 2);
  wait_barrier<TAIL_LOADS>();
  compute(nk - 1);

  float rsum[MT];
#pragma unroll
  for (int i = 0; i < MT; ++i) {
    const int gm = row0 + i * 16 + c16;
    rsum[i] = 0.f;
#pragma unroll
    for (int jp = 0; jp < NP; ++jp) {
      float w[8];
#pragma unroll
      for (int r = 0; r < 4; ++r) {
        const float va = acc[i][2 * jp][r], vb = acc[i][2 * jp + 1][r];
        const auto sw = __builtin_amdgcn_permlane16_swap(__float_as_uint(va), __float_as_uint(vb), false, false);
        w[r] = __uint_as_float(sw[0]) + bias_lo[jp][r];
        w[4 + r] = __uint_as_float(sw[1]) + bias_hi[jp][r];
      }
      const int col = col_of(jp);
      if (p.drop_on) {
        const uint32_t keep = dropout_keep8(rng, (uint64_t)((long)gm * N + col) >> 3, p.thresh);
#pragma unroll
        for (int e = 0; e < 8; ++e) w[e] = ((keep >> e) & 1u) ? w[e] * p.dscale : 0.f;
      }
#pragma unroll
      for (int e = 0; e < 8; ++e) w[e] += (float)res[i][jp][e];
      const bf16x8 zb = pack8(w);
      if (gm < p.M) *reinterpret_cast<bf16x8*>(p.Z + (long)gm * N + col) = zb;
#pragma unroll
      for (int r = 0; r < 4; ++r) {
        const float lo = (float)zb[r], hi = (float)zb[4 + r];
        acc[i][2 * jp][r] = lo;
        acc[i][2 * jp + 1][r] = hi;
        rsum[i] += lo + hi;
      }
    }
    rsum[i] += __shfl_xor(rsum[i], 16, 64);
    rsum[i] += __shfl_xor(rsum[i], 32, 64);
  }
  float* red = reinterpret_cast<float*>(smem);
  __builtin_amdgcn_s_barrier();
  asm volatile("" ::: "memory");
  if (g == 0) {
#pragma unroll
    for (int i = 0; i < MT; ++i) red[wn * BMT + wm * (BMT / 2) + i * 16 + c16] = rsum[i];
  }
  asm volatile("s_waitcnt lgkmcnt(0)" ::: "memory");
  __builtin_amdgcn_s_barrier();
  asm volatile("" ::: "memory");
  float mean[MT], rstd[MT];
  const float invD = 1.0f / (float)N;
#pragma unroll
  for (int i = 0; i < MT; ++i) {
    mean[i] = (rsum[i] + red[(1 - wn) * BMT + wm * (BMT / 2) + i * 16 + c16]) * invD;
// ... 195 lines not shown
  bool rowok[MT];
  f32x4 bias_lo[NP], bias_hi[NP];
  bf16x8 res[MT][NP];
#pragma unroll
  for (int i = 0; i < MT; ++i) rowok[i] = i < gcount && row0 + i * 16 + c16 < r1;
#pragma unroll
  for (int jp = 0; jp < NP; ++jp) {
    const int col = col_of(jp);
    bias_lo[jp] = *reinterpret_cast<const f32x4*>(p.bias + col);
    bias_hi[jp] = *reinterpret_cast<const f32x4*>(p.bias + col + 4);
#pragma unroll
    for (int i = 0; i < MT; ++i) {
      const int gm = min(row0 + i * 16 + c16, r1 - 1);
      res[i][jp] = *reinterpret_cast<const bf16x8*>(p.residual + (long)gm * p.ldr + col);
    }
  }
  float rsum[MT];
#pragma unroll
  for (int i = 0; i < MT; ++i) {
    const int gm = row0 + i * 16 + c16;
    rsum[i] = 0.f;
#pragma unroll
    for (int jp = 0; jp < NP; ++jp) {
      float w[8];
#pragma unroll
      for (int r = 0; r < 4; ++r) {
        const float va = acc[i][2 * jp][r], vb = acc[i][2 * jp + 1][r];
        const auto sw = __builtin_amdgcn_permlane16_swap(__float_as_uint(va), __float_as_uint(vb), false, false);
        w[r] = __uint_as_float(sw[0]) + bias_lo[jp][r];
        w[4 + r] = __uint_as_float(sw[1]) + bias_hi[jp][r];
      }
      const int col = col_of(jp);
      if (p.drop_on) {
        const uint32_t keep = dropout_keep8(rng, (uint64_t)((long)gm * N + col) >> 3, p.thresh);
#pragma unroll
        for (int e = 0; e < 8; ++e) w[e] = ((keep >> e) & 1u) ? w[e] * p.dscale : 0.f;
      }
#pragma unroll
      for (int e = 0; e < 8; ++e) w[e] += (float)res[i][jp][e];
      const bf16x8 zb = pack8(w);
      if (rowok[i]) *reinterpret_cast<bf16x8*>(p.Z + (long)gm * N + col) = zb;
#pragma unroll
      for (int r = 0; r < 4; ++r) {
        const float lo = (float)zb[r], hi = (float)zb[4 + r];
        acc[i][2 * jp][r] = lo;
        acc[i][2 * jp + 1][r] = hi;
        rsum[i] += lo + hi;
      }
    }
    rsum[i] += __shfl_xor(rsum[i], 16, 64);
    rsum[i] += __shfl_xor(rsum[i], 32, 64);
  }
  float* red = reinterpret_cast<float*>(smem);
  if (g == 0) {
#pragma unroll
    for (int i = 0; i < MT; ++i) red[wn * BMT + wm * 64 + i * 16 + c16] = rsum[i];
  }
  asm volatile("s_waitcnt lgkmcnt(0)" ::: "memory");
  __builtin_amdgcn_s_barrier();
  asm volatile("" ::: "memory");
  float mean[MT], rstd[MT];
  const float invD = 1.0f / (float)N;
#pragma unroll
  for (int i = 0; i < MT; ++i) {
    mean[i] = (rsum[i] + red[(1 - wn) * BMT + wm * 64 + i * 16 + c16]) * invD;
    float qv = 0.f;
#pragma unroll
// ... 103 lines not shown
```

### vit-vs-raw-iq_amd/csrc/gemm_lnbwd.hip

```cpp
#include <stdlib.h>

#include "common.h"
#include "gemm_common.h"
#include "gemm_ring.h"
#include "iqvit.h"
#include "prof.h"

namespace {

constexpr int LB_THREADS = 256;

struct LnBwdParams {
  const bf16* A; const bf16* B; const bf16* residual;
  int lda, ldb, ldr, M, K;
  const bf16* Z; const float* mean; const float* rstd; const float* gamma;
  bf16* dZ; bf16* dY;
  float* partial;
  int drop_on; IqRng rng; uint32_t thresh; float dscale;
};

template <int BMT, int BN>
__global__ __launch_bounds__(LB_THREADS, 2) void gemm_lnbwd_kernel(const LnBwdParams p) {
  using Ring = RingShape<BMT, BN>;
  constexpr int BK2 = Ring::BK2, NS = Ring::NS, STAGE_BYTES = Ring::STAGE_BYTES, WN = Ring::WN, NT = Ring::NT, NP = NT / 2, MT = Ring::MT;
// ... 187 lines not shown
    const bool ok = row < p.M;
    const float mean = side[rl], rstd = side[BMT + rl];
    float xh[NV][8], dy[NV][8];
    float s1 = 0.f, s2 = 0.f;
#pragma unroll
    for (int v = 0; v < NV; ++v) {
      bf16x8 td = *reinterpret_cast<const bf16x8*>(img + rl * LDI + (v * LPR + lj) * 8);
      bf16x8 tz = zr[it][v];
      if (!ok) { td = bf16x8{}; tz = bf16x8{}; }
      unpack8(tz, xh[v]);
      unpack8(td, dy[v]);
#pragma unroll
      for (int e = 0; e < 8; ++e) {
        xh[v][e] = ok ? (xh[v][e] - mean) * rstd : 0.f;
        ag[v][e] += dy[v][e] * xh[v][e];
        ab[v][e] += dy[v][e];
        dy[v][e] *= gmm[v][e];
        s1 += dy[v][e];
        s2 += dy[v][e] * xh[v][e];
      }
    }
#pragma unroll
    for (int o = LPR / 2; o > 0; o >>= 1) { s1 += __shfl_xor(s1, o, 64); s2 += __shfl_xor(s2, o, 64); }
    const float c1 = s1 * invD, c2 = s2 * invD;
    if (ok) {
#pragma unroll
      for (int v = 0; v < NV; ++v) {
        float o[8];
#pragma unroll
        for (int e = 0; e < 8; ++e) o[e] = rstd * (dy[v][e] - c1 - xh[v][e] * c2);
        const long off = row * N + (v * LPR + lj) * 8;
        *reinterpret_cast<bf16x8*>(p.dZ + off) = pack8(o);
        if (p.drop_on) {
          const uint32_t keep = dropout_keep8(rng, (uint64_t)off >> 3, p.thresh);
#pragma unroll
          for (int e = 0; e < 8; ++e) o[e] = ((keep >> e) & 1u) ? o[e] * p.dscale : 0.f;
          *reinterpret_cast<bf16x8*>(p.dY + off) = pack8(o);
        }
      }
    }
  }
  float* red = reinterpret_cast<float*>(smem);
  asm volatile("s_waitcnt lgkmcnt(0)" ::: "memory");
  __builtin_amdgcn_s_barrier();
  asm volatile("" ::: "memory");
  const int rslot = wave * RPW + rsub;
#pragma unroll
  for (int v = 0; v < NV; ++v) {
    const int c = (v * LPR + lj) * 8;
#pragma unroll
    for (int e = 0; e < 8; ++e) {
      red[rslot * 2 * N + c + e] = ag[v][e];
      red[rslot * 2 * N + N + c + e] = ab[v][e];
    }
  }
  asm volatile("s_waitcnt lgkmcnt(0)" ::: "memory");
  __builtin_amdgcn_s_barrier();
  asm volatile("" ::: "memory");
  for (int c = tid; c < 2 * N; c += LB_THREADS) {
    float sum = 0.f;
    for (int r = 0; r < RPB; ++r) sum += red[r * 2 * N + c];
    p.partial[(long)blockIdx.x * 2 * N + c] = sum;
  }
}

template <int BMT, int BN>
int launch(const LnBwdParams& p, hipStream_t st) {
// ... 45 lines not shown
```

### vit-vs-raw-iq_amd/csrc/layernorm.hip

```cpp
#include "common.h"
#include "iqvit.h"
#include "prof.h"

namespace {

template <int LPR>
__device__ __forceinline__ float group_sum(float v) {
#pragma unroll
  for (int o = LPR / 2; o > 0; o >>= 1) v += __shfl_xor(v, o, 64);
  return v;
}

constexpr int LN_THREADS = 256;

template <int LPR, int NV, bool MASK = false>
__global__ __launch_bounds__(LN_THREADS) void ln_fwd_kernel(const bf16* __restrict__ Z, const float* __restrict__ gamma,
                                                            const float* __restrict__ beta, bf16* __restrict__ X,
                                                            float* __restrict__ mean_out, float* __restrict__ rstd_out,
                                                            int M, int D, float eps) {
  constexpr int RPW = 64 / LPR;
  constexpr int RPB = RPW * (LN_THREADS / 64);
  const int lane = threadIdx.x & 63, wave = threadIdx.x >> 6;
  const int j = lane % LPR, rsub = lane / LPR;
  float g[NV][8], b[NV][8];
// ... 68 lines not shown
    float s1 = 0.f, s2 = 0.f;
#pragma unroll
    for (int v = 0; v < NV; ++v) {
      bf16x8 tz = {}, td = {};
      const bool cv = !MASK || (v * LPR + j) * 8 < D;
      if (ok && cv) {
        tz = *reinterpret_cast<const bf16x8*>(Z + row * D + (v * LPR + j) * 8);
        td = *reinterpret_cast<const bf16x8*>(dX + row * D + (v * LPR + j) * 8);
      }
      unpack8(tz, xh[v]);
      unpack8(td, dy[v]);
#pragma unroll
      for (int e = 0; e < 8; ++e) {
        xh[v][e] = cv ? (xh[v][e] - mean) * rstd : 0.f;
        ag[v][e] += dy[v][e] * xh[v][e];
        ab[v][e] += dy[v][e];
        dy[v][e] *= g[v][e];
        s1 += dy[v][e];
        s2 += dy[v][e] * xh[v][e];
      }
    }
    const float c1 = group_sum<LPR>(s1) * invD;
    const float c2 = group_sum<LPR>(s2) * invD;
    if (ok) {
#pragma unroll
      for (int v = 0; v < NV; ++v) {
        float o[8];
#pragma unroll
        for (int e = 0; e < 8; ++e) o[e] = rstd * (dy[v][e] - c1 - xh[v][e] * c2);
        const long off = row * D + (v * LPR + j) * 8;
        if (MASK && (v * LPR + j) * 8 >= D) continue;
        *reinterpret_cast<bf16x8*>(dZ + off) = pack8(o);
        if (DROP) {
          const uint32_t keep = dropout_keep8(rng, (uint64_t)off >> 3, thresh);
#pragma unroll
          for (int e = 0; e < 8; ++e) o[e] = ((keep >> e) & 1u) ? o[e] * dscale : 0.f;
          *reinterpret_cast<bf16x8*>(dY + off) = pack8(o);
        }
      }
    }
  }
  const int rslot = wave * RPW + rsub;
#pragma unroll
  for (int v = 0; v < NV; ++v) {
    const int c = (v * LPR + j) * 8;
    if (MASK && c >= D) continue;
#pragma unroll
    for (int e = 0; e < 8; ++e) {
      red[rslot * 2 * D + c + e] = ag[v][e];
      red[rslot * 2 * D + D + c + e] = ab[v][e];
    }
  }
  __syncthreads();
  for (int c = threadIdx.x; c < 2 * D; c += LN_THREADS) {
    float s = 0.f;
    for (int r = 0; r < RPB; ++r) s += red[r * 2 * D + c];
    partial[(long)blockIdx.x * 2 * D + c] = s;
  }
}

__global__ __launch_bounds__(1024) void ln_bwd_reduce_kernel(const float* __restrict__ partial, int nblk, int D,
                                                             float* __restrict__ dgamma, float* __restrict__ dbeta,
                                                             int accumulate) {
  __shared__ float sm[32][33];
  const int cl = threadIdx.x & 31, sl = threadIdx.x >> 5;
  const int c = blockIdx.x * 32 + cl;
  float s = 0.f;
// ... 155 lines not shown
```

### vit-vs-raw-iq_amd/csrc/misc.hip

```cpp
#include "common.h"
#include "iqvit.h"
#include "prof.h"

namespace {

__global__ void patchify_kernel(const float* __restrict__ src, bf16* __restrict__ dst, int kind, int B, int C, int H,
                                int W, int p, int tok, int P, int Kpad) {
  const long nchunk = (long)B * tok * (Kpad / 8);
  for (long id = (long)blockIdx.x * blockDim.x + threadIdx.x; id < nchunk; id += (long)gridDim.x * blockDim.x) {
    const int ch = (int)(id % (Kpad / 8));
    const long row = id / (Kpad / 8);
    const int b = (int)(row / tok), t = (int)(row % tok);
    float v[8];
    if (kind == 0 && (p & 7) == 0 && (W & 3) == 0 && ch * 8 < P) {
      const int k = ch * 8, gw = W / p;
      const int c = k / (p * p), rem = k % (p * p), py = rem / p, px = rem % p;
      const int gy = t / gw, gx = t % gw;
      const float* sp = src + (((long)b * C + c) * H + gy * p + py) * W + gx * p + px;
      const f32x4 a = *reinterpret_cast<const f32x4*>(sp), bq = *reinterpret_cast<const f32x4*>(sp + 4);
      v[0] = a[0]; v[1] = a[1]; v[2] = a[2]; v[3] = a[3]; v[4] = bq[0]; v[5] = bq[1]; v[6] = bq[2]; v[7] = bq[3];
      *reinterpret_cast<bf16x8*>(dst + row * Kpad + ch * 8) = pack8(v);
      continue;
    }
#pragma unroll
// ... 502 lines not shown
  if (b > (size_t)cap) b = cap;
  if (b < 1) b = 1;
  return (int)b;
}

}

extern "C" int iq_patchify(const float* src, void* patches, int kind, int B, int C, int H, int W, int p, int Kpad,
                           iq_stream_t stream) {
  IQ_PROF(IQ_FAM_MISC, stream);
  if (B <= 0) return IQ_OK;
  if (!src || !patches || C <= 0 || H <= 0 || p <= 0 || (Kpad % 8)) return IQ_ERR_ARG;
  int tok, P;
  if (kind == 0) {
    if (W <= 0) return IQ_ERR_ARG;
    tok = (H / p) * (W / p); P = C * p * p;
  } else if (kind == 1) {
    tok = H / p; P = C * p;
  } else {
    return IQ_ERR_ARG;
  }
  if (tok <= 0 || Kpad < P) return IQ_ERR_ARG;
  const size_t n = (size_t)B * tok * (Kpad / 8);
  patchify_kernel<<<grid_for(n, 256, 4096), 256, 0, (hipStream_t)stream>>>(src, (bf16*)patches, kind, B, C, H, W, p, tok,
                                                                          P, Kpad);
  return iq_launch_status();
}

extern "C" int iq_cls_rows(const float* cls, const float* pe, void* x0, int B, int S, int D, const iq_dropout_t* drop,
                           iq_stream_t stream) {
  IQ_PROF(IQ_FAM_MISC, stream);
  if (B <= 0) return IQ_OK;
  if (!cls || !pe || !x0 || (D % 8)) return IQ_ERR_ARG;
  int on; IqRng r; uint32_t th; float sc;
  (void)dropout_unpack(drop, &on, &r, &th, &sc);
  const int n = B * (D / 8);
  cls_rows_kernel<<<(n + 255) / 256, 256, 0, (hipStream_t)stream>>>(cls, pe, (bf16*)x0, B, S, D, on, r, th, sc);
  return iq_launch_status();
}

extern "C" int iq_embed_bwd_gather(const void* dx0, void* demb, float* dcls, int B, int S, int tok, int D, int has_cls,
                                   const iq_dropout_t* drop, int accumulate, iq_stream_t stream) {
  IQ_PROF(IQ_FAM_MISC, stream);
  if (B <= 0) return IQ_OK;
  if (!dx0 || !demb || (D % 8) || (has_cls && !dcls)) return IQ_ERR_ARG;
  int on; IqRng r; uint32_t th; float sc;
  (void)dropout_unpack(drop, &on, &r, &th, &sc);
  const size_t n = (size_t)B * tok * (D / 8);
  hipStream_t st = (hipStream_t)stream;
  embed_bwd_gather_kernel<<<grid_for(n, 256, 4096), 256, 0, st>>>((const bf16*)dx0, (bf16*)demb, B, S, tok, D,
                                                                  has_cls ? 1 : 0, on, r, th, sc);
  if (has_cls) dcls_kernel<<<D / 8, 256, 0, st>>>((const bf16*)dx0, dcls, B, S, D, on, r, th, sc, accumulate);
  return iq_launch_status();
}

extern "C" int iq_head_fwd(const void* x, const float* ln_g, const float* ln_b, const float* W, const float* b,
                           float* featn, float* hstat, float* logits, int B, int S, int D, int K, int pool,
                           iq_stream_t stream) {
  IQ_PROF(IQ_FAM_MISC, stream);
  if (B <= 0) return IQ_OK;
  if (!x || !W || !b || !featn || !logits || (ln_g && (!ln_b || !hstat))) return IQ_ERR_ARG;
  head_fwd_kernel<<<B, 64, 0, (hipStream_t)stream>>>((const bf16*)x, ln_g, ln_b, W, b, featn, hstat, logits, S, D, K, pool);
  return iq_launch_status();
}

extern "C" int iq_ce_fwd_bwd(const float* logits, const int64_t* labels, int B, int K, float smoothing, float denom,
                             float* loss_sum, int32_t* n_correct, float* dlogits, iq_stream_t stream) {
  IQ_PROF(IQ_FAM_MISC, stream);
  if (B <= 0) return IQ_OK;
  if (!logits || !labels || K <= 0 || denom <= 0.f) return IQ_ERR_ARG;
  if (K <= 32) ce_kernel<32><<<1, 256, 0, (hipStream_t)stream>>>(logits, labels, B, K, smoothing, denom, loss_sum, n_correct, dlogits);
  else ce_kernel<0><<<1, 256, 0, (hipStream_t)stream>>>(logits, labels, B, K, smoothing, denom, loss_sum, n_correct, dlogits);
  return iq_launch_status();
}

extern "C" int iq_head_bwd(const float* dlogits, const float* featn, const float* hstat, const float* ln_g,
                           const float* ln_b, const float* W, float* dW, float* db, float* dln_g, float* dln_b,
                           void* dx, int B, int S, int D, int K, int pool, int accumulate, iq_stream_t stream) {
// ... 67 lines not shown
    const float2 v = *reinterpret_cast<const float2*>(raw + (f * len + t) * 2);
    out[f * 2 * take + t] = (v.x - i_mean) / i_std;
    out[f * 2 * take + take + t] = (v.y - q_mean) / q_std;
  }
}

extern "C" int iq_frames_preprocess(const float* raw, float* out, int n_frames, int len, int take, const float* stats,
                                    iq_stream_t stream) {
  if (n_frames <= 0) return IQ_OK;
  if (!raw || !out || !stats || len <= 0 || take <= 0 || take > len) return IQ_ERR_ARG;
  if (!(stats[1] > 0.f) || !(stats[3] > 0.f)) return IQ_ERR_ARG;
  if ((uintptr_t)raw & 7) return IQ_ERR_ARG;
  hipStream_t st = (hipStream_t)stream;
  IQ_PROF(IQ_FAM_MISC, st);
  const long n = (long)n_frames * take;
  long nb = (n + 255) / 256;
  if (nb > 8192) nb = 8192;
  frames_preprocess_kernel<<<(int)nb, 256, 0, st>>>(raw, out, n, len, take, stats[0], stats[1], stats[2], stats[3]);
  return iq_launch_status();
}

int head_bwd_dx_launch(const float* dlogits, const float* featn, const float* hstat, const float* ln_g, const float* W, void* dx,
                       int B, int S, int D, int K, int pool, hipStream_t st) {
  IQ_PROF(IQ_FAM_MISC, st);
  if (B <= 0) return IQ_OK;
  head_bwd_dx_kernel<<<B, 256, D * sizeof(float), st>>>(dlogits, featn, hstat, ln_g, W, (bf16*)dx, S, D, K, pool);
  return iq_launch_status();
}

int embed_bwd_gather_launch(const void* dx0, void* demb, int B, int S, int tok, int D, int has_cls, const iq_dropout_t* drop,
                            hipStream_t st) {
  IQ_PROF(IQ_FAM_MISC, st);
  if (B <= 0) return IQ_OK;
  int on; IqRng r; uint32_t th; float sc;
  (void)dropout_unpack(drop, &on, &r, &th, &sc);
  const size_t n = (size_t)B * tok * (D / 8);
  embed_bwd_gather_kernel<<<grid_for(n, 256, 4096), 256, 0, st>>>((const bf16*)dx0, (bf16*)demb, B, S, tok, D, has_cls ? 1 : 0,
                                                                  on, r, th, sc);
  return iq_launch_status();
}

__global__ __launch_bounds__(256) void linf_step_kernel(float* __restrict__ x, const float* __restrict__ g, const float* __restrict__ x0,
                                                        float alpha, float eps, float lo, float hi, int has_lo, int has_hi, long n) {
  for (long i = (long)blockIdx.x * blockDim.x + threadIdx.x; i < n; i += (long)gridDim.x * blockDim.x) {
    const float gv = g[i];
    const float s = gv > 0.f ? 1.f : gv < 0.f ? -1.f : 0.f;
    float v = __fadd_rn(x[i], __fmul_rn(alpha, s));
    const float c = x0[i];
    v = fminf(fmaxf(v, __fsub_rn(c, eps)), __fadd_rn(c, eps));
    if (has_lo) v = fmaxf(v, lo);
    if (has_hi) v = fminf(v, hi);
    x[i] = v;
  }
}

extern "C" int iq_linf_step(float* x_adv, const float* grad, const float* x0, float alpha, float eps, float lo, float hi, size_t n,
                            iq_stream_t stream) {
  if (!x_adv || !grad || !x0) return IQ_ERR_ARG;
  if (!(alpha >= 0.f) || !(eps >= 0.f) || !(alpha < INFINITY) || !(eps < INFINITY)) return IQ_ERR_ARG;
  const bool has_lo = lo == lo, has_hi = hi == hi;
  if (has_lo && has_hi && lo > hi) return IQ_ERR_ARG;
  if (n == 0) return IQ_OK;
  hipStream_t st = (hipStream_t)stream;
  IQ_PROF(IQ_FAM_MISC, st);
  linf_step_kernel<<<grid_for(n, 256, 8192), 256, 0, st>>>(x_adv, grad, x0, alpha, eps, lo, hi, has_lo ? 1 : 0, has_hi ? 1 : 0,
                                                           (long)n);
// ... 3 lines not shown
```

### vit-vs-raw-iq_amd/csrc/model.hip

```cpp
#include <hip/hip_runtime.h>
#include <stdio.h>
#include <stdlib.h>
#include <string.h>

#include <string>
#include <vector>

#include "attn_maps.h"
#include "common.h"
#include "iqvit.h"
#include "prof.h"

int head_bwd_dx_launch(const float* dlogits, const float* featn, const float* hstat, const float* ln_g, const float* W, void* dx,
                       int B, int S, int D, int K, int pool, hipStream_t st);
int embed_bwd_gather_launch(const void* dx0, void* demb, int B, int S, int tok, int D, int has_cls, const iq_dropout_t* drop,
                            hipStream_t st);

namespace {

struct Entry {
  std::string name;
  size_t off;
  int ndim;
  int dims[4];
};

struct LayerOff {
  size_t wqkv, bqkv, wo, bo, g1, be1, w1, b1, w2, b2, g2, be2, end;
  size_t t_wqkv, t_wo, t_w1, t_w2;
};

inline size_t align_up(size_t v, size_t a) { return (v + a - 1) / a * a; }

struct WsPlan {
  size_t step_ctr, patches, x0, head_feat, head_stat;
  struct L { size_t qkv, att, lse, z1, mean1, rstd1, x1, hid, gate, z2, mean2, rstd2, x2; };
  std::vector<L> layers;
  size_t gA, gB, gAtt, demb, wgrad_ws, wgrad_ws_bytes, ln_part[2], embw_scratch;
  size_t gZ, gY, gZ1, gY1, gH, gQKV;
  size_t total;
};

__global__ void bf16_to_f32_kernel(const bf16* __restrict__ s, float* __restrict__ d, size_t n8) {
  for (size_t i = (size_t)blockIdx.x * blockDim.x + threadIdx.x; i < n8; i += (size_t)gridDim.x * blockDim.x) {
    const bf16x8 v = reinterpret_cast<const bf16x8*>(s)[i];
    f32x4 a = {(float)v[0], (float)v[1], (float)v[2], (float)v[3]};
    f32x4 b = {(float)v[4], (float)v[5], (float)v[6], (float)v[7]};
    reinterpret_cast<f32x4*>(d)[2 * i] = a;
    reinterpret_cast<f32x4*>(d)[2 * i + 1] = b;
// ... 33 lines not shown
  int e = 0;
  while (e + 1 < nent && (int)blockIdx.x >= tab[e + 1].tile0) ++e;
  const TransDesc d = tab[e];
  const int local = blockIdx.x - d.tile0;
  const int bx = (local % d.tiles_x) * 32, by = (local / d.tiles_x) * 32;
  const float* src = params + d.src_off;
  bf16* dst = reinterpret_cast<bf16*>(shadow + d.dst_off);
  const int tx = threadIdx.x & 31, ty = threadIdx.x >> 5;
  for (int i = ty; i < 32; i += 8) {
    const int r = by + i, c = bx + tx;
    t[i][tx] = (r < d.rows && c < d.cols) ? src[(long)r * d.cols + c] : 0.f;
  }
  __syncthreads();
  for (int i = ty; i < 32; i += 8) {
    const int c = bx + i, r = by + tx;
    if (c < d.cols && r < d.rows) dst[(long)c * d.rows + r] = (bf16)t[tx][i];
  }
}

__global__ void rel_start_kernel(float* r, int n, int S, int cls) {
  for (int i = blockIdx.x * blockDim.x + threadIdx.x; i < n; i += gridDim.x * blockDim.x) {
    const int k = i % S;
    r[i] = cls ? (k == 0 ? 1.f : 0.f) : 1.0f / S;
  }
}

struct RelHook {
  float* const* maps;
  int rows, heads, positive;
  long bstride;
  float* rel;
  float* r[2];
};

__global__ void set_u32_kernel(uint32_t* p, uint32_t v, int bump) {
  if (threadIdx.x == 0 && blockIdx.x == 0) *p = bump ? *p + 1u : v;
}

inline int blocks_for(size_t n, int cap = 4096) {
  size_t b = (n + 255) / 256;
  if (b > (size_t)cap) b = cap;
  if (b < 1) b = 1;
  return (int)b;
}

}

struct iq_model {
  iq_model_cfg_t c;
  int S, tok, has_cls, P, Ppad, dh, pool, head_ln;
  std::vector<Entry> entries;
  size_t nparam;
  size_t emb_w, emb_b, cls, emb_end;
  std::vector<LayerOff> L;
  size_t hln_g, hln_b, head_w, head_b, head_begin;
  size_t sh_flat, sh_embw, sh_table, shadow_bytes;
  std::vector<TransDesc> ttab;
  int ttiles = 0;
  const void* table_uploaded_to = nullptr;
  float* params = nullptr;
  float* grads = nullptr;
  const float* pe = nullptr;
  unsigned char* shadow = nullptr;
  std::string err;
  uint32_t* step_ctr = nullptr;
  uint64_t last_seed = 0;
  bool last_tr = false;
  bool last_train_fwd = false;
  const void* fwd_ws = nullptr;
  int fwd_batch = 0;

  iq_dropout_t bwd_site(uint32_t id, const uint32_t* step_dev, bool tr) const {
    iq_dropout_t d;
    d.seed = last_seed; d.step = 0; d.site = id; d.p = tr ? c.drop_prob : 0.f; d.step_dev = step_dev;
    return d;
  }

  size_t add(const std::string& name, std::vector<int> dims, size_t& cur, bool aligned = true) {
    if (aligned) cur = align_up(cur, 64);
    Entry e;
    e.name = name; e.off = cur; e.ndim = (int)dims.size();
    size_t n = 1;
    for (int i = 0; i < 4; ++i) { e.dims[i] = i < e.ndim ? dims[i] : 1; n *= (size_t)e.dims[i]; }
    entries.push_back(e);
    cur += n;
    return e.off;
  }
  const bf16* sh(size_t off) const { return reinterpret_cast<const bf16*>(shadow + sh_flat) + off; }
  const bf16* sht(size_t byte_off) const { return reinterpret_cast<const bf16*>(shadow + byte_off); }
};

namespace {

int fail(iq_model* m, int code, const std::string& msg) {
  if (m) m->err = msg;
  return code;
}

WsPlan plan_ws(const iq_model* m, int B) {
  WsPlan w;
  const size_t D = m->c.d_model, F = m->c.ffn_hidden, S = m->S, H = m->c.n_head;
  const size_t M = (size_t)B * S, MT = (size_t)B * m->tok;
  size_t cur = 0;
  auto take = [&](size_t bytes) { size_t o = cur; cur = align_up(cur + bytes, 256); return o; };
  w.step_ctr = take(256);
  w.patches = take(MT * m->Ppad * 2);
  w.x0 = take(M * D * 2);
// ... 6 lines not shown
    l.lse = take((size_t)B * H * S * 4);
    l.z1 = take(M * D * 2);
    l.mean1 = take(M * 4);
    l.rstd1 = take(M * 4);
    l.x1 = take(M * D * 2);
    l.hid = take(M * F * 2);
    l.gate = take(iq_ffn_chain_gate_bytes((int)M, (int)F));
    l.z2 = take(M * D * 2);
    l.mean2 = take(M * 4);
    l.rstd2 = take(M * 4);
    l.x2 = take(M * D * 2);
  }
  w.gA = take(M * D * 2);
  w.gB = take(M * D * 2);
  w.gZ = take(M * D * 2);
  w.gY = take(M * D * 2);
  w.gZ1 = take(M * D * 2);
  w.gY1 = take(M * D * 2);
  w.gH = take(M * F * 2);
  w.gQKV = take(M * 3 * D * 2);
  w.gAtt = take(M * D * 2);
  w.demb = take(MT * D * 2);
  size_t wb = 0;
  auto mx = [&](size_t v) { if (v > wb) wb = v; };
  {
    iq_wgrad_problem_t g[4];
    memset(g, 0, sizeof(g));
    g[0].N = (int)D; g[0].K = (int)F;
    g[1].N = (int)F; g[1].K = (int)D;
    g[2].N = (int)D; g[2].K = (int)D;
    g[3].N = (int)(3 * D); g[3].K = (int)D;
    mx(iq_wgrad_grouped_ws_bytes(g, 4, (int)M, 0));
    for (int k = 0; k < 4; ++k) mx(iq_wgrad_grouped_ws_bytes(g + k, 1, (int)M, 0));
  }
  mx(iq_wgrad_ws_bytes((int)MT, (int)D, m->Ppad));
  w.wgrad_ws_bytes = wb;
  w.wgrad_ws = take(wb);
  size_t ln_rows_fused = (size_t)iq_gemm_lnbwd_partial_rows((int)M);
  if ((size_t)iq_ffn_chain_bwd_partial_rows((int)M) > ln_rows_fused) ln_rows_fused = (size_t)iq_ffn_chain_bwd_partial_rows((int)M);
  ln_rows_fused *= 2 * D * sizeof(float);
  const size_t ln_bytes = ln_rows_fused > iq_ln_bwd_ws_bytes((int)D) ? ln_rows_fused : iq_ln_bwd_ws_bytes((int)D);
  for (int k = 0; k < 2; ++k) w.ln_part[k] = take(ln_bytes);
  w.embw_scratch = take((size_t)D * m->Ppad * 4 + 256);
  w.total = cur;
  return w;
}

inline bool use_fused_ln(int D, int K) { return iq_gemm_ln_supported(D, K) && (D <= 192 || K <= 256); }

inline bool use_ffn_chain(int M, int S, int D, int F) {
  static const int tune = [] { const char* e = getenv("IQ_TUNE_FFN_CHAIN"); return e ? atoi(e) : -1; }();
  static const int min_rows = [] { const char* e = getenv("IQ_TUNE_FFN_CHAIN_MIN_ROWS"); return e ? atoi(e) : 8192; }();
  if (!iq_ffn_chain_supported(S, D, F) || tune == 0) return false;
  if (tune == 1) return true;
  return M >= min_rows;
}

inline int use_chain_pre(int M) {
  static const int tune = [] { const char* e = getenv("IQ_TUNE_CHAIN_PRE"); return e ? atoi(e) : -1; }();
  return tune >= 0 ? tune : M <= 32768 ? 3 : 2;
}

#define IQ_TRY(expr, what)                                                              \
  do {                                                                                  \
    int rc_ = (expr);                                                                   \
    if (rc_ != IQ_OK) return fail(m, rc_, std::string(what) + " failed (status " + std::to_string(rc_) + ")"); \
  } while (0)

iq_dropout_t site(const iq_model* m, uint64_t seed, const uint32_t* step_dev, uint32_t id, bool training) {
  iq_dropout_t d;
  d.seed = seed; d.step = 0; d.site = id; d.p = training ? m->c.drop_prob : 0.f; d.step_dev = step_dev;
  return d;
}

}

extern "C" int iq_model_create(const iq_model_cfg_t* cfg, iq_model_t** out) {
  if (!cfg || !out) return IQ_ERR_ARG;
  *out = nullptr;
  iq_model* m = new iq_model();
  m->c = *cfg;
  const iq_model_cfg_t& c = m->c;
  auto bad = [&](const char* msg) { fprintf(stderr, "iq_model_create: %s\n", msg); delete m; return IQ_ERR_UNSUPPORTED; };
  if (c.d_model <= 0 || c.n_head <= 0 || c.n_layers < 0 || c.ffn_hidden <= 0 || c.num_classes <= 0 || c.in_channels <= 0)
    { delete m; return IQ_ERR_ARG; }
  if (c.d_model % c.n_head) return bad("d_model must be divisible by n_head");
  m->dh = c.d_model / c.n_head;
  if (m->dh != 16 && m->dh != 32 && m->dh != 64) return bad("head dim (d_model/n_head) must be 16, 32 or 64");
  if (c.ffn_hidden % 8) return bad("ffn_hidden must be a multiple of 8");
  if (!iq_ln_supported(c.d_model)) return bad("d_model not supported by the LayerNorm kernel");
  if (!(c.drop_prob >= 0.f && c.drop_prob < 1.f)) return bad("drop_prob must be in [0,1)");
  if (c.kind == 0) {
    if (c.patch <= 0 || c.img_h < c.patch || c.img_w < c.patch) return bad("bad image / patch size");
    m->tok = (c.img_h / c.patch) * (c.img_w / c.patch);
    m->has_cls = 1;
    m->P = c.in_channels * c.patch * c.patch;
    m->pool = 0;
    m->head_ln = 0;
  } else if (c.kind == 1) {
    if (c.conv_k <= 0 || c.seq_length < c.conv_k || (c.seq_length % c.conv_k)) return bad("bad seq_length / segment_size");
    m->tok = c.seq_length / c.conv_k;
    m->has_cls = c.use_cls ? 1 : 0;
    m->P = c.in_channels * c.conv_k;
    m->pool = m->has_cls ? 0 : 1;
// ... 126 lines not shown

static int refresh_impl(iq_model_t* m, bool cast_flat, iq_stream_t stream) {
  if (!m || !m->params || !m->shadow) return fail(m, IQ_ERR_ARG, "refresh_shadow: model not bound");
  hipStream_t st = (hipStream_t)stream;
  const int D = m->c.d_model;
  if (cast_flat) IQ_TRY(iq_cast_bf16(m->params, m->shadow + m->sh_flat, m->nparam, stream), "cast params");
  IQ_PROF(IQ_FAM_MISC, st);
  cast_pad_kernel<<<blocks_for((size_t)D * m->Ppad), 256, 0, st>>>(m->params + m->emb_w, (bf16*)(m->shadow + m->sh_embw), D,
                                                                  m->P, m->Ppad);
  if (m->ttiles > 0)
    transpose_table_kernel<<<m->ttiles, 256, 0, st>>>(m->params, m->shadow, (const TransDesc*)(m->shadow + m->sh_table),
                                                     (int)m->ttab.size());
  return iq_launch_status();
}

extern "C" int iq_model_refresh_shadow(iq_model_t* m, iq_stream_t stream) { return refresh_impl(m, true, stream); }
extern "C" int iq_model_refresh_transposed(iq_model_t* m, iq_stream_t stream) { return refresh_impl(m, false, stream); }

extern "C" int iq_model_forward(iq_model_t* m, const float* src, int batch, void* workspace, size_t ws_bytes,
                                int training, uint64_t seed, uint32_t step, float* enc_out, float* logits,
                                iq_stream_t stream) {
  if (!m) return IQ_ERR_ARG;
  if (!m->params || !m->shadow || !m->pe) return fail(m, IQ_ERR_ARG, "forward: model not bound");
  if (!src || !workspace || batch <= 0) return fail(m, IQ_ERR_ARG, "forward: bad arguments");
  if ((uintptr_t)workspace & 255) return fail(m, IQ_ERR_ARG, "forward: workspace must be 256 B aligned");
  const WsPlan w = plan_ws(m, batch);
  if (ws_bytes < w.total) return fail(m, IQ_ERR_ARG, "forward: workspace too small");
  hipStream_t st = (hipStream_t)stream;
  unsigned char* ws = (unsigned char*)workspace;
  const iq_model_cfg_t& c = m->c;
  const int D = c.d_model, F = c.ffn_hidden, S = m->S, H = c.n_head, B = batch;
  const int M = B * S, MT = B * m->tok;
  const bool tr = training != 0 && c.drop_prob > 0.f;
  uint32_t* step_dev = m->step_ctr ? m->step_ctr : (uint32_t*)(ws + w.step_ctr);
  m->last_tr = tr;
  m->last_train_fwd = true;
  if (tr) {
    set_u32_kernel<<<1, 64, 0, st>>>(step_dev, step, step == 0xFFFFFFFFu ? 1 : 0);
    m->last_seed = seed;
  }
  const float* P = m->params;
  m->fwd_ws = nullptr;

  if (c.kind == 0) IQ_TRY(iq_patchify(src, ws + w.patches, 0, B, c.in_channels, c.img_h, c.img_w, c.patch, m->Ppad, stream), "patchify");
  else IQ_TRY(iq_patchify(src, ws + w.patches, 1, B, c.in_channels, c.seq_length, 0, c.conv_k, m->Ppad, stream), "patchify");
  const iq_dropout_t d0 = site(m, seed, step_dev, 0, tr);
  if (m->has_cls) IQ_TRY(iq_cls_rows(P + m->cls, m->pe, ws + w.x0, B, S, D, &d0, stream), "cls rows");
  {
    iq_epilogue_t e;
    memset(&e, 0, sizeof(e));
    e.bias = P + m->emb_b; e.pe = m->pe; e.tok = m->tok; e.seq = S; e.cls_off = m->has_cls; e.drop = d0;
    IQ_TRY(iq_gemm_bf16_nt(ws + w.patches, m->Ppad, m->shadow + m->sh_embw, m->Ppad, ws + w.x0, D, MT, D, m->Ppad, &e, stream),
           "embedding GEMM");
  }
  const unsigned char* x = ws + w.x0;
  bool qkv_done = false;
  for (int l = 0; l < c.n_layers; ++l) {
    const LayerOff& o = m->L[l];
    const WsPlan::L& a = w.layers[l];
    iq_epilogue_t e;
    if (!qkv_done) {
      memset(&e, 0, sizeof(e));
      e.bias = P + o.bqkv;
      IQ_TRY(iq_gemm_bf16_nt(x, D, m->sh(o.wqkv), D, ws + a.qkv, 3 * D, M, 3 * D, D, &e, stream), "qkv GEMM");
    }
    qkv_done = false;
    IQ_TRY(iq_attn_fwd(ws + a.qkv, ws + a.att, (float*)(ws + a.lse), B, S, H, m->dh, stream), "attention fwd");
    const iq_dropout_t dr1 = site(m, seed, step_dev, 1 + 3 * l, tr);
    const iq_dropout_t drh = site(m, seed, step_dev, 2 + 3 * l, tr);
    const iq_dropout_t dr2 = site(m, seed, step_dev, 3 + 3 * l, tr);
    if (use_ffn_chain(M, S, D, F) && use_chain_pre(M)) {
      const bool next = l + 1 < c.n_layers && use_chain_pre(M) >= 2;
      IQ_TRY(iq_attn_out_ffn_chain_fwd(ws + a.att, m->sh(o.wo), P + o.bo, &dr1, x, P + o.g1, P + o.be1, ws + a.z1, ws + a.x1,
                                       (float*)(ws + a.mean1), (float*)(ws + a.rstd1), m->sh(o.w1), P + o.b1, &drh, ws + a.hid,
                                       m->sh(o.w2), P + o.b2, &dr2, P + o.g2, P + o.be2, 1e-12f, ws + a.z2, ws + a.x2,
                                       (float*)(ws + a.mean2), (float*)(ws + a.rstd2), ws + a.gate,
                                       next ? m->sh(m->L[l + 1].wqkv) : nullptr, next ? P + m->L[l + 1].bqkv : nullptr,
                                       next ? ws + w.layers[l + 1].qkv : nullptr, B, S, D, F, stream),
             "out-proj + norm1 + ffn chain + norm2 (+ next q,k,v)");
      qkv_done = next;
      x = ws + a.x2;
      continue;
    }
    if (use_fused_ln(D, D)) {
      IQ_TRY(iq_gemm_bf16_ln(ws + a.att, D, m->sh(o.wo), D, P + o.bo, x, D, &dr1, P + o.g1, P + o.be1, 1e-12f, ws + a.z1,
                             ws + a.x1, (float*)(ws + a.mean1), (float*)(ws + a.rstd1), M, D, D, stream), "out-proj GEMM + norm1");
    } else {
      memset(&e, 0, sizeof(e));
      e.bias = P + o.bo; e.drop = dr1; e.residual = x; e.ldr = D;
      IQ_TRY(iq_gemm_bf16_nt(ws + a.att, D, m->sh(o.wo), D, ws + a.z1, D, M, D, D, &e, stream), "out-proj GEMM");
      IQ_TRY(iq_ln_fwd(ws + a.z1, P + o.g1, P + o.be1, ws + a.x1, (float*)(ws + a.mean1), (float*)(ws + a.rstd1), M, D, 1e-12f, stream), "norm1");
    }
    if (use_ffn_chain(M, S, D, F)) {
      IQ_TRY(iq_ffn_chain_fwd(ws + a.x1, m->sh(o.w1), P + o.b1, &drh, ws + a.hid, m->sh(o.w2), P + o.b2, &dr2, P + o.g2, P + o.be2,
                              1e-12f, ws + a.z2, ws + a.x2, (float*)(ws + a.mean2), (float*)(ws + a.rstd2), ws + a.gate, B, S, D, F, stream),
             "ffn chain + norm2");
    } else {
      memset(&e, 0, sizeof(e));
      e.bias = P + o.b1; e.relu = 1; e.drop = drh;
      IQ_TRY(iq_gemm_bf16_nt(ws + a.x1, D, m->sh(o.w1), D, ws + a.hid, F, M, F, D, &e, stream), "ffn1 GEMM");
      if (use_fused_ln(D, F)) {
        IQ_TRY(iq_gemm_bf16_ln(ws + a.hid, F, m->sh(o.w2), F, P + o.b2, ws + a.x1, D, &dr2, P + o.g2, P + o.be2, 1e-12f,
                               ws + a.z2, ws + a.x2, (float*)(ws + a.mean2), (float*)(ws + a.rstd2), M, D, F, stream), "ffn2 GEMM + norm2");
      } else {
        memset(&e, 0, sizeof(e));
        e.bias = P + o.b2; e.drop = dr2; e.residual = ws + a.x1; e.ldr = D;
        IQ_TRY(iq_gemm_bf16_nt(ws + a.hid, F, m->sh(o.w2), F, ws + a.z2, D, M, D, F, &e, stream), "ffn2 GEMM");
        IQ_TRY(iq_ln_fwd(ws + a.z2, P + o.g2, P + o.be2, ws + a.x2, (float*)(ws + a.mean2), (float*)(ws + a.rstd2), M, D, 1e-12f, stream), "norm2");
      }
    }
    x = ws + a.x2;
  }
  if (logits) {
    IQ_TRY(iq_head_fwd(x, m->head_ln ? P + m->hln_g : nullptr, m->head_ln ? P + m->hln_b : nullptr, P + m->head_w,
                       P + m->head_b, (float*)(ws + w.head_feat), (float*)(ws + w.head_stat), logits, B, S, D,
                       c.num_classes, m->pool, stream), "head");
  }
  if (enc_out) bf16_to_f32_kernel<<<blocks_for((size_t)M * D / 8), 256, 0, st>>>((const bf16*)x, enc_out, (size_t)M * D / 8);
  const int rc = iq_launch_status();
  if (rc == IQ_OK) { m->fwd_ws = workspace; m->fwd_batch = batch; }
  return rc;
}

static int maps_check(iq_model_t* m, const void* workspace, size_t ws_bytes, int batch, const char* what, WsPlan* w) {
  if (!workspace || batch <= 0) return fail(m, IQ_ERR_ARG, std::string(what) + ": bad arguments");
  if (!m->fwd_ws) return fail(m, IQ_ERR_ARG, std::string(what) + ": no forward has run in a workspace");
  if (m->fwd_ws != workspace) return fail(m, IQ_ERR_ARG, std::string(what) + ": the last forward ran in another workspace");
  if (m->fwd_batch != batch)
    return fail(m, IQ_ERR_ARG, std::string(what) + ": the last forward in this workspace had batch " + std::to_string(m->fwd_batch) +
                                   ", not " + std::to_string(batch));
  *w = plan_ws(m, batch);
  if (ws_bytes < w->total) return fail(m, IQ_ERR_ARG, std::string(what) + ": workspace too small");
  return IQ_OK;
}

extern "C" int iq_model_attention(iq_model_t* m, const void* workspace, size_t ws_bytes, int batch, int layer, int rows,
                                  int heads, float* out, long out_bstride, iq_stream_t stream) {
  if (!m) return IQ_ERR_ARG;
  WsPlan w;
  const int rc = maps_check(m, workspace, ws_bytes, batch, "attention", &w);
  if (rc != IQ_OK) return rc;
  if (layer < 0 || layer >= m->c.n_layers) return fail(m, IQ_ERR_ARG, "attention: layer index out of range");
  if (rows < 0 || rows > 2 || heads < 0 || heads > 1) return fail(m, IQ_ERR_ARG, "attention: rows must be 0, 1 or 2 and heads 0 or 1");
  if (!out) return fail(m, IQ_ERR_ARG, "attention: out is NULL");
  const int S = m->S, H = m->c.n_head;
  if (out_bstride < (long)(heads ? 1 : H) * S * (rows == 0 ? S : 1)) return fail(m, IQ_ERR_ARG, "attention: out_bstride too small");
  const unsigned char* ws = (const unsigned char*)workspace;
  const WsPlan::L& a = w.layers[layer];
  IQ_TRY(iq_attn_probs(ws + a.qkv, (const float*)(ws + a.lse), out, out_bstride, batch, S, H, m->dh, rows, heads, stream),
         "attention probabilities");
  return IQ_OK;
}

extern "C" int iq_model_attention_rollout(iq_model_t* m, const void* workspace, size_t ws_bytes, int batch, float alpha,
                                          float* out, iq_stream_t stream) {
  if (!m) return IQ_ERR_ARG;
  WsPlan w;
  const int rc = maps_check(m, workspace, ws_bytes, batch, "attention rollout", &w);
  if (rc != IQ_OK) return rc;
  if (!(alpha >= 0.f && alpha <= 1.f)) return fail(m, IQ_ERR_ARG, "attention rollout: alpha must be in [0, 1]");
  if (!out) return fail(m, IQ_ERR_ARG, "attention rollout: out is NULL");
  const unsigned char* ws = (const unsigned char*)workspace;
  const int L = m->c.n_layers;
// ... 9 lines not shown
}

extern "C" int iq_model_grad_range(const iq_model_t* m, int stage_hi, int stage_lo, size_t* off, size_t* len) {
  if (!m || !off || !len) return IQ_ERR_ARG;
  const int Lr = m->c.n_layers;
  if (stage_lo < 0 || stage_hi > Lr + 1 || stage_lo > stage_hi) return IQ_ERR_ARG;
  auto begin = [&](int s) { return s == 0 ? (size_t)0 : (s <= Lr ? (s == 1 ? m->emb_end : m->L[s - 2].end) : m->head_begin); };
  auto end = [&](int s) { return s == 0 ? m->emb_end : (s <= Lr ? m->L[s - 1].end : m->nparam); };
  *off = begin(stage_lo);
  *len = end(stage_hi) - *off;
  return IQ_OK;
}

static int backward_impl(iq_model_t* m, const float* dlogits, const float* denc, int batch, void* workspace, size_t ws_bytes,
                         int accumulate, int stage_hi, int stage_lo, bool pgrads, iq_stream_t stream,
                         const RelHook* rh = nullptr) {
  if (!m->params || (pgrads && !m->grads) || !m->shadow) return fail(m, IQ_ERR_ARG, "backward: model not bound (grads required)");
  if (!workspace || batch <= 0) return fail(m, IQ_ERR_ARG, "backward: bad arguments");
  const iq_model_cfg_t& c = m->c;
  const int Lr = c.n_layers;
  if (stage_lo < 0 || stage_hi > Lr + 1 || stage_lo > stage_hi) return fail(m, IQ_ERR_ARG, "backward: bad stage range");
  const WsPlan w = plan_ws(m, batch);
  if (ws_bytes < w.total) return fail(m, IQ_ERR_ARG, "backward: workspace too small");
  hipStream_t st = (hipStream_t)stream;
  unsigned char* ws = (unsigned char*)workspace;
  const int D = c.d_model, F = c.ffn_hidden, S = m->S, H = c.n_head, B = batch, K = c.num_classes;
  const int M = B * S, MT = B * m->tok;
  const bool tr = m->last_tr;
  const uint32_t* step_dev = m->step_ctr ? m->step_ctr : (const uint32_t*)(ws + w.step_ctr);
  const float* P = m->params;
  float* G = m->grads;
  float* wws = (float*)(ws + w.wgrad_ws);
  const float dscale = tr ? dropout_scale(c.drop_prob) : 1.f;

  if (stage_hi == Lr + 1) {
    if (!dlogits && !denc) return fail(m, IQ_ERR_ARG, "backward: dlogits or denc required at the head stage");
    if (dlogits && !pgrads) {
      IQ_TRY(head_bwd_dx_launch(dlogits, (const float*)(ws + w.head_feat), (const float*)(ws + w.head_stat),
                                m->head_ln ? P + m->hln_g : nullptr, P + m->head_w, ws + w.gA, B, S, D, K, m->pool, st), "head bwd (dx)");
    } else if (dlogits) {
      IQ_TRY(iq_head_bwd(dlogits, (const float*)(ws + w.head_feat), (const float*)(ws + w.head_stat),
                         m->head_ln ? P + m->hln_g : nullptr, m->head_ln ? P + m->hln_b : nullptr, P + m->head_w,
                         G + m->head_w, G + m->head_b, m->head_ln ? G + m->hln_g : nullptr,
                         m->head_ln ? G + m->hln_b : nullptr, ws + w.gA, B, S, D, K, m->pool, accumulate, stream), "head bwd");
    } else if (!accumulate && pgrads) {
      (void)hipMemsetAsync(G + m->head_begin, 0, (m->nparam - m->head_begin) * sizeof(float), st);
    }
    if (denc) f32_into_bf16_kernel<<<blocks_for((size_t)M * D / 8), 256, 0, st>>>(denc, (bf16*)(ws + w.gA), (size_t)M * D / 8, dlogits ? 1 : 0);
  }
  const bool fuse1 = iq_gemm_lnbwd_supported(D, F) != 0, fuse2 = iq_gemm_lnbwd_supported(D, 3 * D) != 0;
  bool deferred = false;
  for (int sidx = (stage_hi > Lr ? Lr : stage_hi); sidx >= 1 && sidx >= stage_lo; --sidx) {
    const int l = sidx - 1;
    const LayerOff& o = m->L[l];
    const WsPlan::L& a = w.layers[l];
    const unsigned char* xin = l == 0 ? ws + w.x0 : ws + w.layers[l - 1].x2;
    unsigned char *gZ = ws + w.gZ, *gY = ws + w.gY, *gZ1 = ws + w.gZ1, *gY1 = ws + w.gY1;
    unsigned char *gH = ws + w.gH, *gQKV = ws + w.gQKV;
    iq_epilogue_t e;
    float* lp2 = (float*)(ws + w.ln_part[0]);
    float* lp1 = (float*)(ws + w.ln_part[1]);
    const bool norm2_here = l == Lr - 1 || !fuse2;
    if (norm2_here) {
      const iq_dropout_t dr2 = m->bwd_site(3 + 3 * l, step_dev, tr);
      IQ_TRY(iq_ln_bwd(ws + w.gA, ws + a.z2, (const float*)(ws + a.mean2), (const float*)(ws + a.rstd2), P + o.g2,
                       gZ, gY, &dr2, nullptr, nullptr, lp2, accumulate, M, D, stream), "norm2 bwd");
    }
    const unsigned char* dO2 = tr ? gY : gZ;
    const unsigned char* dAo = tr ? gY1 : gZ1;
    const iq_wgrad_problem_t wg[4] = {
        {dO2, D, ws + a.hid, F, G + o.w2, G + o.b2, D, F},
        {gH, F, ws + a.x1, D, G + o.w1, G + o.b1, F, D},
        {dAo, D, ws + a.att, D, G + o.wo, G + o.bo, D, D},
        {gQKV, 3 * D, xin, D, G + o.wqkv, G + o.bqkv, 3 * D, D}};
    const int rows2 = norm2_here ? iq_ln_bwd_partial_rows(M, D) : deferred ? iq_ffn_chain_bwd_partial_rows(M) : iq_gemm_lnbwd_partial_rows(M);
    const bool chain = fuse1 && m->last_train_fwd && use_ffn_chain(M, S, D, F);
    const int rows1 = chain ? iq_ffn_chain_bwd_partial_rows(M) : fuse1 ? iq_gemm_lnbwd_partial_rows(M) : iq_ln_bwd_partial_rows(M, D);
    const iq_reduce_seg_t lnseg[4] = {{lp2, rows2, 2L * D, G + o.g2, D}, {lp2 + D, rows2, 2L * D, G + o.be2, D},
                                      {lp1, rows1, 2L * D, G + o.g1, D}, {lp1 + D, rows1, 2L * D, G + o.be1, D}};
    const iq_dropout_t dr1 = m->bwd_site(1 + 3 * l, step_dev, tr);
    const bool post = chain && use_chain_pre(M) >= 2;
    if (chain && deferred) {
      const LayerOff& ou = m->L[l + 1];
      const iq_dropout_t dr2b = m->bwd_site(3 + 3 * l, step_dev, tr);
      IQ_TRY(iq_qkv_dgrad_ffn_chain_bwd(gQKV, m->sht(ou.t_wqkv), gZ1, ws + a.z2, (const float*)(ws + a.mean2), (const float*)(ws + a.rstd2),
                                        P + o.g2, &dr2b, gZ, gY, lp2, m->sht(o.t_w2), ws + a.gate, dscale, gH, m->sht(o.t_w1), gZ, ws + a.z1,
                                        (const float*)(ws + a.mean1), (const float*)(ws + a.rstd1), P + o.g1, &dr1, gZ1, gY1, lp1,
                                        m->sht(o.t_wo), ws + w.gAtt, B, S, D, F, stream),
             "qkv dgrad of the layer above + norm2 bwd + ffn chain bwd + norm1 bwd + out-proj dgrad");
    } else if (chain) {
      IQ_TRY(iq_ffn_chain_bwd(dO2, m->sht(o.t_w2), ws + a.gate, dscale, gH, m->sht(o.t_w1), gZ, ws + a.z1, (const float*)(ws + a.mean1),
                              (const float*)(ws + a.rstd1), P + o.g1, &dr1, gZ1, gY1, lp1, post ? m->sht(o.t_wo) : nullptr,
                              post ? ws + w.gAtt : nullptr, B, S, D, F, stream), "ffn chain bwd + norm1 bwd (+ out-proj dgrad)");
    } else {
      memset(&e, 0, sizeof(e));
      e.gate = ws + a.hid; e.ldg = F; e.gate_scale = dscale;
      IQ_TRY(iq_gemm_bf16_nt(dO2, D, m->sht(o.t_w2), D, gH, F, M, F, D, &e, stream), "ffn2 dgrad");
      if (fuse1) {
        IQ_TRY(iq_gemm_bf16_lnbwd(gH, F, m->sht(o.t_w1), F, gZ, D, ws + a.z1, (const float*)(ws + a.mean1),
                                  (const float*)(ws + a.rstd1), P + o.g1, &dr1, gZ1, gY1, lp1, M, D, F, stream), "ffn1 dgrad + norm1 bwd");
      } else {
        memset(&e, 0, sizeof(e));
        e.residual = gZ; e.ldr = D;
        IQ_TRY(iq_gemm_bf16_nt(gH, F, m->sht(o.t_w1), F, ws + w.gB, D, M, D, F, &e, stream), "ffn1 dgrad");
        IQ_TRY(iq_ln_bwd(ws + w.gB, ws + a.z1, (const float*)(ws + a.mean1), (const float*)(ws + a.rstd1), P + o.g1,
                         gZ1, gY1, &dr1, nullptr, nullptr, lp1, accumulate, M, D, stream), "norm1 bwd");
      }
    }
    if (!post) IQ_TRY(iq_gemm_bf16_nt(dAo, D, m->sht(o.t_wo), D, ws + w.gAtt, D, M, D, D, nullptr, stream), "out-proj dgrad");
    if (rh) {
      const float* lse = (const float*)(ws + a.lse);
      if (rh->maps && rh->maps[l])
        IQ_TRY(iq_attn_grad_probs(ws + a.qkv, lse, ws + w.gAtt, rh->maps[l], rh->bstride, B, S, H, m->dh, rh->rows, rh->heads,
                                  rh->positive, stream), "gradient-weighted attention map");
      if (rh->rel) {
        const int i = Lr - 1 - l;
        IQ_TRY(attn_relevance_step_launch(ws + a.qkv, lse, ws + w.gAtt, i ? rh->r[(i - 1) & 1] : nullptr, l ? rh->r[i & 1] : rh->rel,
                                          B, S, H, m->dh, i ? 0 : m->has_cls ? 1 : 2, st), "relevance step");
      }
      if (l == 0) break;
    }
    IQ_TRY(iq_attn_bwd(ws + a.qkv, ws + a.att, ws + w.gAtt, (const float*)(ws + a.lse), gQKV, B, S, H, m->dh, stream), "attention bwd");
    if (pgrads) IQ_TRY(iq_gemm_bf16_wgrad_grouped(wg, 4, M, wws, w.wgrad_ws_bytes, accumulate, 0, lnseg, 4, stream), "layer weight gradients");
    deferred = l > 0 && fuse2 && chain && post && use_chain_pre(M) >= 3 && sidx - 1 >= stage_lo;
    if (deferred) continue;
    if (l > 0 && fuse2) {
      const LayerOff& ob = m->L[l - 1];
      const WsPlan::L& ab = w.layers[l - 1];
      const iq_dropout_t dr2b = m->bwd_site(3 + 3 * (l - 1), step_dev, tr);
      IQ_TRY(iq_gemm_bf16_lnbwd(gQKV, 3 * D, m->sht(o.t_wqkv), 3 * D, gZ1, D, ws + ab.z2, (const float*)(ws + ab.mean2),
                                (const float*)(ws + ab.rstd2), P + ob.g2, &dr2b, gZ, gY, lp2, M, D, 3 * D, stream),
             "qkv dgrad + norm2 bwd of the layer below");
    } else {
      memset(&e, 0, sizeof(e));
      e.residual = gZ1; e.ldr = D;
      IQ_TRY(iq_gemm_bf16_nt(gQKV, 3 * D, m->sht(o.t_wqkv), 3 * D, ws + w.gA, D, M, D, 3 * D, &e, stream), "qkv dgrad");
    }
  }
  if (stage_lo == 0) {
    const iq_dropout_t dr0 = m->bwd_site(0, step_dev, tr);
    if (!pgrads) {
      IQ_TRY(embed_bwd_gather_launch(ws + w.gA, ws + w.demb, B, S, m->tok, D, m->has_cls, &dr0, st), "embedding bwd gather");
      return iq_launch_status();
    }
    IQ_TRY(iq_embed_bwd_gather(ws + w.gA, ws + w.demb, m->has_cls ? G + m->cls : nullptr, B, S, m->tok, D, m->has_cls,
                               &dr0, accumulate, stream), "embedding bwd gather");
    if (m->Ppad == m->P) {
      IQ_TRY(iq_gemm_bf16_wgrad(ws + w.demb, D, ws + w.patches, m->Ppad, G + m->emb_w, G + m->emb_b, MT, D, m->Ppad, wws,
                                w.wgrad_ws_bytes, accumulate, stream), "embedding wgrad");
    } else {
      float* scratch = (float*)(ws + w.embw_scratch);
      if (accumulate) (void)hipMemsetAsync(scratch, 0, (size_t)D * m->Ppad * sizeof(float), st);
      IQ_TRY(iq_gemm_bf16_wgrad(ws + w.demb, D, ws + w.patches, m->Ppad, scratch, G + m->emb_b, MT, D, m->Ppad, wws,
                                w.wgrad_ws_bytes, accumulate, stream), "embedding wgrad");
// ... 65 lines not shown
```

### vit-vs-raw-iq_amd/trainer.py

```python
from __future__ import annotations

import ctypes as C
import math
from typing import List, Optional, Sequence, Tuple

import torch
import torch.distributed as dist

from . import _native as N
from .modules import NativePlan


def make_buckets(n_layers: int, n_buckets: int) -> List[Tuple[int, int]]:
    stages = list(range(n_layers + 1, -1, -1))
    n_buckets = max(1, min(n_buckets, len(stages)))
    per = math.ceil(len(stages) / n_buckets)
    out = []
    for i in range(0, len(stages), per):
        chunk = stages[i:i + per]
        out.append((chunk[0], chunk[-1]))
    return out


class BucketReducer:
# ... 103 lines not shown
                sl["graphs"] = None
        elif self._slot is not None:
            self._slot["graphs"] = value

    def _buffers(self, B: int):
        if self._batch != B:
            sl = self._slots.pop(B, None)
            if sl is None:
                K = self.plan.cfg.num_classes
                sl = {"logits": torch.empty(B, K, dtype=torch.float32, device=self.device),
                      "dlogits": torch.empty(B, K, dtype=torch.float32, device=self.device),
                      "static": None, "graphs": None, "captured": None}
                while len(self._slots) >= self.MAX_SLOTS:
                    self._slots.pop(next(iter(self._slots)))
            self._slots[B] = sl
            self._slot = sl
            self._logits, self._dlogits = sl["logits"], sl["dlogits"]
            self._batch = B
        self.plan.workspace(B, self.device)

    def _pointers(self):
        p = self.plan
        return (p.ws.data_ptr(), p.ws.numel(), p.flat.data_ptr(), p.shadow.data_ptr(), p.step_ctr.data_ptr(),
                self._logits.data_ptr(), self._dlogits.data_ptr(), self.gflat.data_ptr(), self._batch)

    def _segments(self, x: torch.Tensor, y: torch.Tensor, auto_step: bool):
        plan, L = self.plan, self.L
        B = x.shape[0]
        ws = plan.ws
        step_arg = 0xFFFFFFFF if auto_step else (self.steps + 1) & 0x7FFFFFFF

        def fwd_and_first_bucket():
            st = N.stream_handle()
            N.check(L.iq_model_forward(plan.h, x.data_ptr(), B, ws.data_ptr(), ws.numel(), 1, plan.seed, step_arg, None,
                                       self._logits.data_ptr(), st), "iq_model_forward", plan.h)
            N.check(L.iq_ce_fwd_bwd(self._logits.data_ptr(), y.data_ptr(), B, plan.cfg.num_classes, self.smoothing,
                                    float(B), self.loss_sum.data_ptr(), self.n_correct.data_ptr(),
                                    self._dlogits.data_ptr(), st), "iq_ce_fwd_bwd")
            bwd(0)()

        def bwd(i):
            hi, lo = self.buckets[i]

            def run():
                N.check(L.iq_model_backward(plan.h, self._dlogits.data_ptr(), None, B, ws.data_ptr(), ws.numel(), 0, hi,
                                            lo, N.stream_handle()), "iq_model_backward", plan.h)
            return run

        def optimizer():
            st = N.stream_handle()
            gscale = 1.0 / self.world
            N.check(L.iq_gradnorm_sq(self.gflat.data_ptr(), plan.nparam, gscale, self.gn_ws.data_ptr(),
                                     self.gnorm_sq.data_ptr(), st), "iq_gradnorm_sq")
            N.check(L.iq_counter_add(None, 0, self.dyn.data_ptr() + 4, 1.0, st), "iq_counter_add")
            N.check(L.iq_adamw_step(plan.flat.data_ptr(), self.gflat.data_ptr(), self.exp_avg.data_ptr(),
                                    self.exp_avg_sq.data_ptr(), plan.shadow.data_ptr(), plan.nparam, self.lr,
                                    self.betas[0], self.betas[1], self.eps, self.wd, 0, self.gnorm_sq.data_ptr(),
                                    self.max_norm, gscale, self.dyn.data_ptr(), st), "iq_adamw_step")
            N.check(L.iq_model_refresh_transposed(plan.h, st), "iq_model_refresh_transposed", plan.h)

        return [fwd_and_first_bucket] + [bwd(i) for i in range(1, len(self.buckets))] + [optimizer]

    def _run_segments(self, runners):
        nb = len(self.buckets)
        for i, run in enumerate(runners):
            if i == nb:
                self.reducer.wait()
            run()
# ... 83 lines not shown
```

Before: 53040 frames/s.

## Compute only CLS rows in the top encoder layer for logits-only training

Adds a logits-only forward mode in which the last transformer layer computes attention queries, out-projection, norms and FFN for the CLS token rows only, since a CLS-pooled head reads nothing else. The matching backward runs attention bwd with a single query tile, does the dgrad and wgrad GEMMs over B rows instead of B*S, and scatters the CLS gradient back into the dense residual gradient. The trainer now requests this mode. This removes roughly one layer's worth of per-token FFN and projection work in both forward and backward, at the cost of new special-case kernels, an extra dropout row-indexing field, and guards against dense-output use.

New measurement: 53360 frames/s (median of 6 runs). No clear change (+0.6%).

```diff
diff --git a/include/iqvit.h b/include/iqvit.h
--- a/include/iqvit.h
+++ b/include/iqvit.h
@@ -16,6 +16,7 @@
   uint32_t step;
   uint32_t site;
   float p;
+  uint32_t row_mul;
   const uint32_t* step_dev;
 } iq_dropout_t;
 #define IQ_SITE_IMPAIR 0xFFFFFFFFu
@@ -107,6 +108,9 @@
 int iq_attn_fwd(const void* qkv, void* out, float* lse, int B, int S, int H, int dh, iq_stream_t stream);
 int iq_attn_bwd(const void* qkv, const void* out, const void* dout, const float* lse, void* dqkv, int B, int S, int H,
                 int dh, iq_stream_t stream);
+int iq_attn_fwd_cls(const void* qkv, void* out, float* lse, int B, int S, int H, int dh, iq_stream_t stream);
+int iq_attn_bwd_cls(const void* qkv, const void* out, const void* dout, const float* lse, void* dqkv, int B, int S, int H,
+                    int dh, iq_stream_t stream);
 int iq_attn_fwd_masked(const void* qkv, void* out, float* lse, const uint8_t* mask, long mask_hstride, int B, int S,
                        int H, int dh, iq_stream_t stream);
 int iq_attn_bwd_masked(const void* qkv, const void* out, const void* dout, const float* lse, void* dqkv,
@@ -199,6 +203,8 @@
 int iq_model_bind_step_counter(iq_model_t* m, uint32_t* counter);
 int iq_model_refresh_shadow(iq_model_t* m, iq_stream_t stream);
 int iq_model_refresh_transposed(iq_model_t* m, iq_stream_t stream);
+#define IQ_FWD_TRAIN 1
+#define IQ_FWD_LOGITS_ONLY 2
 int iq_model_forward(iq_model_t* m, const float* src, int batch, void* workspace, size_t ws_bytes, int training,
                      uint64_t seed, uint32_t step, float* enc_out, float* logits, iq_stream_t stream);
 int iq_model_backward(iq_model_t* m, const float* dlogits, const float* denc, int batch, void* workspace,
diff --git a/vit-vs-raw-iq_amd/_native.py b/vit-vs-raw-iq_amd/_native.py
--- a/vit-vs-raw-iq_amd/_native.py
+++ b/vit-vs-raw-iq_amd/_native.py
@@ -7,6 +7,8 @@
 LIB_PATH = os.environ.get("IQ_LIBIQVIT") or os.path.join(_HERE, "libiqvit.so")
 
 BWD_PARAM_GRADS = 1
+FWD_TRAIN = 1
+FWD_LOGITS_ONLY = 2
 
 STATUS = {0: "ok", 1: "invalid argument", 2: "unsupported shape/configuration", 3: "HIP launch error"}
 
@@ -17,7 +19,7 @@
 
 class Dropout(C.Structure):
     _fields_ = [("seed", C.c_uint64), ("step", C.c_uint32), ("site", C.c_uint32), ("p", C.c_float),
-                ("step_dev", C.c_void_p)]
+                ("row_mul", C.c_uint32), ("step_dev", C.c_void_p)]
 
 
 class Impair(C.Structure):
@@ -93,6 +95,8 @@
     "iq_attn_supported": (_I, [_I, _I]),
     "iq_attn_fwd": (_I, [_P, _P, _P, _I, _I, _I, _I, _P]),
     "iq_attn_bwd": (_I, [_P, _P, _P, _P, _P, _I, _I, _I, _I, _P]),
+    "iq_attn_fwd_cls": (_I, [_P, _P, _P, _I, _I, _I, _I, _P]),
+    "iq_attn_bwd_cls": (_I, [_P, _P, _P, _P, _P, _I, _I, _I, _I, _P]),
     "iq_attn_fwd_masked": (_I, [_P, _P, _P, _P, C.c_long, _I, _I, _I, _I, _P]),
     "iq_attn_bwd_masked": (_I, [_P, _P, _P, _P, _P, _P, C.c_long, _I, _I, _I, _I, _P]),
     "iq_attn_probs": (_I, [_P, _P, _P, C.c_long, _I, _I, _I, _I, _I, _I, _P]),
diff --git a/vit-vs-raw-iq_amd/csrc/attention.hip b/vit-vs-raw-iq_amd/csrc/attention.hip
--- a/vit-vs-raw-iq_amd/csrc/attention.hip
+++ b/vit-vs-raw-iq_amd/csrc/attention.hip
@@ -106,7 +106,7 @@
 __global__ __launch_bounds__(ATT_THREADS) void attn_fwd_kernel(const bf16* __restrict__ qkv, bf16* __restrict__ out,
                                                                float* __restrict__ lse, const uint8_t* __restrict__ mask,
                                                                long mask_hstride, int S, int H, int kchunk,
-                                                               float scale_log2, float masked_raw) {
+                                                               float scale_log2, float masked_raw, int qtile_limit) {
   using C = AttCfg<DH>;
   extern __shared__ __attribute__((aligned(16))) unsigned char smem[];
   bf16* Ks = reinterpret_cast<bf16*>(smem);
@@ -119,7 +119,7 @@
   const bf16* kb_ = qb + D;
   const bf16* vb_ = qb + 2 * D;
   const uint8_t* mk = MASKED ? mask + (long)b * (mask_hstride ? (long)H * S * S : (long)S * S) + h * mask_hstride : nullptr;
-  const int qtiles = (S + 31) / 32, npass = (qtiles + ATT_WAVES - 1) / ATT_WAVES, nstage = (S + kchunk - 1) / kchunk;
+  const int qtiles = min((S + 31) / 32, qtile_limit), npass = (qtiles + ATT_WAVES - 1) / ATT_WAVES, nstage = (S + kchunk - 1) / kchunk;
 
   if (nstage == 1) {
     stage_pair<DH, 4>(Ks, kb_, ldg, Vs, vb_, ldg, 0, min(kchunk, ((S + 31) / 32) * 32), S, tid);
@@ -251,7 +251,7 @@
                                                                const bf16* __restrict__ dout, const float* __restrict__ lse,
                                                                bf16* __restrict__ dqkv, const uint8_t* __restrict__ mask,
                                                                long mask_hstride, int S, int H, int spad, int chunk,
-                                                               float scale, float masked_raw) {
+                                                               float scale, float masked_raw, int cls) {
   using C = AttCfg<DH>;
   extern __shared__ __attribute__((aligned(16))) unsigned char smem[];
   bf16* I0 = reinterpret_cast<bf16*>(smem);
@@ -270,21 +270,29 @@
   bf16* dqb = dqkv + (long)b * S * ldg + h * DH;
   const uint8_t* mk = MASKED ? mask + (long)b * (mask_hstride ? (long)H * S * S : (long)S * S) + h * mask_hstride : nullptr;
   const float scale_log2 = scale * LOG2E;
-  const int nblk = spad / 32;
+  const int qpad = cls ? 32 : spad;
+  const int dlive = cls ? 1 : S;
+  const int nblk = qpad / 32;
   const int nchunk = (spad + chunk - 1) / chunk;
+  const int nqchunk = cls ? 1 : nchunk;
   const bool single = nchunk == 1;
 
   if (single) {
-    stage_pair<DH, 4>(I0, qb, ldg, I1, dob, (long)D, 0, spad, S, tid);
+    if (cls) {
+      stage_rows<DH>(I0, qb, ldg, 0, qpad, S, tid);
+      stage_rows<DH>(I1, dob, (long)D, 0, qpad, dlive, tid);
+    } else {
+      stage_pair<DH, 4>(I0, qb, ldg, I1, dob, (long)D, 0, spad, S, tid);
+    }
     __syncthreads();
   }
-  for (int q = tid; q < spad; q += ATT_THREADS) {
+  for (int q = tid; q < qpad; q += ATT_THREADS) {
     float dl = 0.f, ls = 0.f;
     if (q < S) {
 #pragma unroll
       for (int c = 0; c < C::CPR; ++c) {
         const bf16x8 a = single ? *reinterpret_cast<const bf16x8*>(I1 + q * C::LD + c * 8)
-                                : *reinterpret_cast<const bf16x8*>(dob + (long)q * D + c * 8);
+                         : q < dlive ? *reinterpret_cast<const bf16x8*>(dob + (long)q * D + c * 8) : bf16x8{};
         const bf16x8 o8 = *reinterpret_cast<const bf16x8*>(ob + (long)q * D + c * 8);
 #pragma unroll
         for (int e = 0; e < 8; ++e) dl += (float)a[e] * (float)o8[e];
@@ -311,12 +319,17 @@
     for (int dt = 0; dt < C::DT; ++dt) { dv[dt] = f32x4{0.f, 0.f, 0.f, 0.f}; dk[dt] = f32x4{0.f, 0.f, 0.f, 0.f}; }
     const int key = unit * 16 + c16;
     const bool unit_partial = unit * 16 + 16 > S;
-    for (int qc = 0; qc < nchunk; ++qc) {
+    for (int qc = 0; qc < nqchunk; ++qc) {
       const int q0 = qc * chunk;
-      const int rows = min(chunk, spad - q0);
+      const int rows = min(chunk, qpad - q0);
       if (!single) {
         __syncthreads();
-        stage_pair<DH, 2>(I0, qb, ldg, I1, dob, (long)D, q0, rows, S, tid);
+        if (cls) {
+          stage_rows<DH>(I0, qb, ldg, q0, rows, S, tid);
+          stage_rows<DH>(I1, dob, (long)D, q0, rows, dlive, tid);
+        } else {
+          stage_pair<DH, 2>(I0, qb, ldg, I1, dob, (long)D, q0, rows, S, tid);
+        }
         __syncthreads();
       }
       if (!have) continue;
@@ -389,7 +402,7 @@
 #pragma unroll
         for (int s = 0; s < C::KS; ++s) {
           qf[u][s] = row_frag_gmem<DH>(qb, ldg, q, have ? S : 0, s, lane);
-          dof[u][s] = row_frag_gmem<DH>(dob, (long)D, q, have ? S : 0, s, lane);
+          dof[u][s] = row_frag_gmem<DH>(dob, (long)D, q, have ? dlive : 0, s, lane);
         }
       }
       lq[u] = lse_s[q];
@@ -473,6 +486,12 @@
       }
     }
   }
+  if (cls) {
+    for (int id = tid; id < (S - qpad) * C::CPR; id += ATT_THREADS) {
+      const int r = qpad + id / C::CPR, c = id % C::CPR;
+      *reinterpret_cast<bf16x8*>(dqb + (long)r * ldg + c * 8) = bf16x8{};
+    }
+  }
 }
 
 constexpr int ONCE_MAX_SPAD = 224;
@@ -521,14 +540,16 @@
 template <int NT>
 __global__ __launch_bounds__(NT, 4) void attn_bwd_once_kernel(const bf16* __restrict__ qkv, const bf16* __restrict__ out,
                                                               const bf16* __restrict__ dout, const float* __restrict__ lse,
-                                                              bf16* __restrict__ dqkv, int S, int H, int spad, float scale) {
+                                                              bf16* __restrict__ dqkv, int S, int H, int spad, float scale,
+                                                              int cls) {
   constexpr int DH = 64, KS = 2, DT = 4, NW = NT / 64;
   extern __shared__ __attribute__((aligned(16))) unsigned char smem[];
+  const int qpad = cls ? 32 : spad;
   bf16* I0 = reinterpret_cast<bf16*>(smem);
   bf16* I1 = I0 + spad * ONCE_LD;
-  float* lse_s = reinterpret_cast<float*>(I1 + spad * ONCE_LD);
-  float* del_s = lse_s + spad;
-  bf16* dSi = reinterpret_cast<bf16*>(del_s + spad);
+  float* lse_s = reinterpret_cast<float*>(I1 + qpad * ONCE_LD);
+  float* del_s = lse_s + qpad;
+  bf16* dSi = reinterpret_cast<bf16*>(del_s + qpad);
   const int tid = threadIdx.x, lane = tid & 63, wave = tid >> 6, g = lane >> 4, c16 = lane & 15;
   const int b = blockIdx.x / H, h = blockIdx.x % H;
   const int D = H * DH;
@@ -543,14 +564,23 @@
   const int nunit = (S + 15) / 16;
   const int ldS = nunit * 16 + 8;
 
-  {
+  if (cls) {
+    bf16* const imgq[1] = {I0};
+    const bf16* const srcq[1] = {qb};
+    const long ldq[1] = {ldg};
+    once_stage<NT, 2048 / NT, 1>(imgq, srcq, ldq, qpad, S, tid);
+    bf16* const imgd[1] = {I1};
+    const bf16* const srcd[1] = {dob};
+    const long ldd[1] = {(long)D};
+    once_stage<NT, 2048 / NT, 1>(imgd, srcd, ldd, qpad, 1, tid);
+  } else {
     bf16* const img[2] = {I0, I1};
     const bf16* const src[2] = {qb, dob};
     const long lds_[2] = {ldg, (long)D};
     once_stage<NT, 2048 / NT, 2>(img, src, lds_, spad, S, tid);
   }
   __syncthreads();
-  for (int q = tid; q < spad; q += NT) {
+  for (int q = tid; q < qpad; q += NT) {
     float dl = 0.f, ls = 0.f;
     if (q < S) {
 #pragma unroll
@@ -579,7 +609,7 @@
     for (int dt = 0; dt < DT; ++dt) { dv[dt] = f32x4{0.f, 0.f, 0.f, 0.f}; dk[dt] = f32x4{0.f, 0.f, 0.f, 0.f}; }
     const int key = unit * 16 + c16;
     const bool unit_partial = unit * 16 + 16 > S;
-    for (int ql = 0; ql < spad; ql += 32) {
+    for (int ql = 0; ql < qpad; ql += 32) {
       const bool u1 = ql + 16 < S;
       f32x4 p[2], ds[2];
 #pragma unroll
@@ -641,6 +671,13 @@
   __syncthreads();
   for (int half = wave; half < nunit; half += NW) {
     const int q = half * 16 + c16;
+    if (cls && half >= 2) {
+      if (q < S) {
+#pragma unroll
+        for (int dt = 0; dt < DT; ++dt) *reinterpret_cast<bf16x4*>(dqb + (long)q * ldg + dt * 16 + 4 * g) = bf16x4{};
+      }
+      continue;
+    }
     const bf16* drow = dSi + q * ldS + 4 * g;
     f32x4 dq[DT];
 #pragma unroll
@@ -1083,7 +1120,7 @@
 
 template <int DH, bool MASKED>
 int launch_fwd(const void* qkv, void* out, float* lse, const uint8_t* mask, long mask_hstride, int B, int S, int H,
-               hipStream_t st) {
+               hipStream_t st, int qtile_limit = 1 << 30) {
   const int spad = (S + 31) / 32 * 32;
   int kchunk = (int)(ATT_LDS_FWD_BUDGET / (2 * AttCfg<DH>::LD * 2)) / 32 * 32;
   if (kchunk > spad) kchunk = spad;
@@ -1092,13 +1129,13 @@
   if (lds > 48 * 1024)
     (void)hipFuncSetAttribute((const void*)attn_fwd_kernel<DH, MASKED>, hipFuncAttributeMaxDynamicSharedMemorySize, (int)lds);
   attn_fwd_kernel<DH, MASKED><<<B * H, ATT_THREADS, lds, st>>>((const bf16*)qkv, (bf16*)out, lse, mask, mask_hstride, S, H,
-                                                               kchunk, scale_log2, -10000.0f * sqrtf((float)DH));
+                                                               kchunk, scale_log2, -10000.0f * sqrtf((float)DH), qtile_limit);
   return iq_launch_status();
 }
 
 template <int DH, bool MASKED>
 int launch_bwd(const void* qkv, const void* out, const void* dout, const float* lse, void* dqkv, const uint8_t* mask,
-               long mask_hstride, int B, int S, int H, hipStream_t st) {
+               long mask_hstride, int B, int S, int H, hipStream_t st, int cls = 0) {
   const int spad = (S + 31) / 32 * 32;
   const int chunk = bwd_chunk_rows<DH>(S);
   if (S > ATT_MAX_S || chunk < 32) return IQ_ERR_UNSUPPORTED;
@@ -1107,7 +1144,7 @@
     (void)hipFuncSetAttribute((const void*)attn_bwd_kernel<DH, MASKED>, hipFuncAttributeMaxDynamicSharedMemorySize, (int)lds);
   attn_bwd_kernel<DH, MASKED><<<B * H, ATT_THREADS, lds, st>>>((const bf16*)qkv, (const bf16*)out, (const bf16*)dout, lse,
                                                                (bf16*)dqkv, mask, mask_hstride, S, H, spad, chunk,
-                                                               1.0f / sqrtf((float)DH), -10000.0f * sqrtf((float)DH));
+                                                               1.0f / sqrtf((float)DH), -10000.0f * sqrtf((float)DH), cls);
   return iq_launch_status();
 }
 
@@ -1118,13 +1155,13 @@
 }
 template <int NT>
 int launch_bwd_once(const void* qkv, const void* out, const void* dout, const float* lse, void* dqkv, int B, int S, int H,
-                    hipStream_t st) {
-  const int spad = (S + 31) / 32 * 32, nunit = (S + 15) / 16;
-  const size_t lds = (size_t)2 * spad * ONCE_LD * 2 + (size_t)2 * spad * sizeof(float) + (size_t)spad * (nunit * 16 + 8) * 2;
+                    hipStream_t st, int cls = 0) {
+  const int spad = (S + 31) / 32 * 32, nunit = (S + 15) / 16, qpad = cls ? 32 : spad;
+  const size_t lds = (size_t)(spad + qpad) * ONCE_LD * 2 + (size_t)2 * qpad * sizeof(float) + (size_t)qpad * (nunit * 16 + 8) * 2;
   auto k = attn_bwd_once_kernel<NT>;
   if (lds > 48 * 1024) (void)hipFuncSetAttribute((const void*)k, hipFuncAttributeMaxDynamicSharedMemorySize, (int)lds);
   k<<<B * H, NT, lds, st>>>((const bf16*)qkv, (const bf16*)out, (const bf16*)dout, lse, (bf16*)dqkv, S, H, spad,
-                            1.0f / sqrtf(64.0f));
+                            1.0f / sqrtf(64.0f), cls);
   return iq_launch_status();
 }
 
@@ -1149,6 +1186,10 @@
   }
 }
 
+}
+
+int attn_bwd_is_per_frame(int S, int H, int dh) {
+  return (dh == 16 || dh == 32 || dh == 64) && use_frame(S, frame_bwd_lds(S, H, dh)) ? 1 : 0;
 }
 
 extern "C" int iq_attn_supported(int S, int dh) {
@@ -1215,3 +1256,43 @@
                            int S, int H, int dh, iq_stream_t stream) {
   return iq_attn_bwd_masked(qkv, out, dout, lse, dqkv, nullptr, 0, B, S, H, dh, stream);
 }
+
+extern "C" int iq_attn_fwd_cls(const void* qkv, void* out, float* lse, int B, int S, int H, int dh, iq_stream_t stream) {
+  if (B <= 0) return IQ_OK;
+  if (!qkv || !out || !lse || S <= 0 || H <= 0) return IQ_ERR_ARG;
+  hipStream_t st = (hipStream_t)stream;
+  IQ_PROF(IQ_FAM_ATTN_FWD, st);
+  {
+    const double rows = (double)B * S, Dm = (double)H * dh, qr = (double)B * (S < 32 ? S : 32);
+    IQ_PROF_K(2.0 * rows * 2.0 * Dm + 2.0 * qr * 2.0 * Dm + 4.0 * H * qr, 4.0 * H * qr * S * dh, "attn_fwd_kernel<%d, false>", dh);
+  }
+  switch (dh) {
+    case 16: return launch_fwd<16, false>(qkv, out, lse, nullptr, 0, B, S, H, st, 1);
+    case 32: return launch_fwd<32, false>(qkv, out, lse, nullptr, 0, B, S, H, st, 1);
+    case 64: return launch_fwd<64, false>(qkv, out, lse, nullptr, 0, B, S, H, st, 1);
+    default: return IQ_ERR_UNSUPPORTED;
+  }
+}
+
+extern "C" int iq_attn_bwd_cls(const void* qkv, const void* out, const void* dout, const float* lse, void* dqkv, int B,
+                               int S, int H, int dh, iq_stream_t stream) {
+  if (B <= 0) return IQ_OK;
+  if (!qkv || !out || !dout || !lse || !dqkv || S <= 0 || H <= 0) return IQ_ERR_ARG;
+  hipStream_t st = (hipStream_t)stream;
+  IQ_PROF(IQ_FAM_ATTN_BWD, st);
+  const int once = once_threads(S, dh, false);
+  {
+    const double rows = (double)B * S, Dm = (double)H * dh, qr = (double)B * (S < 32 ? S : 32);
+    const double bytes = 2.0 * rows * 6.0 * Dm + 2.0 * qr * 2.0 * Dm + 4.0 * H * qr;
+    if (once) IQ_PROF_K(bytes, 10.0 * H * qr * S * dh, "attn_bwd_once_kernel<%d>", once);
+    else IQ_PROF_K(bytes, 14.0 * H * qr * S * dh, "attn_bwd_kernel<%d, false>", dh);
+  }
+  if (once == 512) return launch_bwd_once<512>(qkv, out, dout, lse, dqkv, B, S, H, st, 1);
+  if (once) return launch_bwd_once<1024>(qkv, out, dout, lse, dqkv, B, S, H, st, 1);
+  switch (dh) {
+    case 16: return launch_bwd<16, false>(qkv, out, dout, lse, dqkv, nullptr, 0, B, S, H, st, 1);
+    case 32: return launch_bwd<32, false>(qkv, out, dout, lse, dqkv, nullptr, 0, B, S, H, st, 1);
+    case 64: return launch_bwd<64, false>(qkv, out, dout, lse, dqkv, nullptr, 0, B, S, H, st, 1);
+    default: return IQ_ERR_UNSUPPORTED;
+  }
+}
diff --git a/vit-vs-raw-iq_amd/csrc/common.h b/vit-vs-raw-iq_amd/csrc/common.h
--- a/vit-vs-raw-iq_amd/csrc/common.h
+++ b/vit-vs-raw-iq_amd/csrc/common.h
@@ -45,6 +45,7 @@
   uint32_t step;
   uint32_t site;
   const uint32_t* step_dev;
+  uint32_t row_mul = 1;
 };
 
 __device__ __forceinline__ IqRng rng_resolve(IqRng r) {
@@ -108,11 +109,12 @@
   *on = 0; *rng = IqRng{0, 0, 0, nullptr}; *thresh = 0; *dscale = 1.f;
   if (!d || !(d->p > 0.f)) return true;
   *on = 1;
-  *rng = IqRng{d->seed, d->step, d->site, d->step_dev};
+  *rng = IqRng{d->seed, d->step, d->site, d->step_dev, d->row_mul > 1 ? d->row_mul : 1u};
   *thresh = dropout_thresh(d->p);
   *dscale = dropout_scale(d->p);
   return d->p < 1.f;
 }
+inline bool dropout_rows_dense(const iq_dropout_t* d) { return !d || !(d->p > 0.f) || d->row_mul <= 1; }
 
 constexpr int vmcnt_imm(int n) { return (n & 15) | ((n >> 4) << 14) | 0x0F70; }
 
diff --git a/vit-vs-raw-iq_amd/csrc/ffn_chain.hip b/vit-vs-raw-iq_amd/csrc/ffn_chain.hip
--- a/vit-vs-raw-iq_amd/csrc/ffn_chain.hip
+++ b/vit-vs-raw-iq_amd/csrc/ffn_chain.hip
@@ -1086,6 +1086,7 @@
   p.gate = (uint32_t*)gate_bits;
   if ((uintptr_t)gate_bits % 16) return IQ_ERR_ARG;
   p.M = frames * S; p.F = F; p.eps = eps;
+  if (!dropout_rows_dense(drop1) || !dropout_rows_dense(drop2) || (pre && !dropout_rows_dense(pre->drop0))) return IQ_ERR_ARG;
   if (!dropout_unpack(drop1, &p.drop1_on, &p.rng1, &p.thresh1, &p.dscale1) ||
       !dropout_unpack(drop2, &p.drop2_on, &p.rng2, &p.thresh2, &p.dscale2)) return IQ_ERR_ARG;
   if (pre) {
@@ -1164,6 +1165,7 @@
   p.gH = (bf16*)gH; p.dZ = (bf16*)dz; p.dY = (bf16*)dy; p.partial = partial;
   p.M = frames * S; p.F = F; p.gate_scale = gate_scale;
   p.Wot = (const bf16*)Wot; p.dA = (bf16*)dA;
+  if (!dropout_rows_dense(drop) || (pre && !dropout_rows_dense(pre->drop0))) return IQ_ERR_ARG;
   if (!dropout_unpack(drop, &p.drop_on, &p.rng, &p.thresh, &p.dscale) || (p.drop_on && !dy)) return IQ_ERR_ARG;
   if (pre) {
     if (!Wot) return IQ_ERR_ARG;
diff --git a/vit-vs-raw-iq_amd/csrc/gemm_common.h b/vit-vs-raw-iq_amd/csrc/gemm_common.h
--- a/vit-vs-raw-iq_amd/csrc/gemm_common.h
+++ b/vit-vs-raw-iq_amd/csrc/gemm_common.h
@@ -132,7 +132,7 @@
           for (int e = 0; e < 4; ++e) { w[e] += pa[e]; w[4 + e] += pb[e]; }
         }
         if (p.drop_on) {
-          const uint32_t keep = dropout_keep8(rng, (uint64_t)(orow * p.N + col) >> 3, p.thresh);
+          const uint32_t keep = dropout_keep8(rng, (uint64_t)(orow * rng.row_mul * p.N + col) >> 3, p.thresh);
 #pragma unroll
           for (int e = 0; e < 8; ++e) w[e] = ((keep >> e) & 1u) ? w[e] * p.dscale : 0.f;
         }
diff --git a/vit-vs-raw-iq_amd/csrc/gemm_ln.hip b/vit-vs-raw-iq_amd/csrc/gemm_ln.hip
--- a/vit-vs-raw-iq_amd/csrc/gemm_ln.hip
+++ b/vit-vs-raw-iq_amd/csrc/gemm_ln.hip
@@ -144,7 +144,7 @@
       }
       const int col = col_of(jp);
       if (p.drop_on) {
-        const uint32_t keep = dropout_keep8(rng, (uint64_t)((long)gm * N + col) >> 3, p.thresh);
+        const uint32_t keep = dropout_keep8(rng, (uint64_t)((long)gm * rng.row_mul * N + col) >> 3, p.thresh);
 #pragma unroll
         for (int e = 0; e < 8; ++e) w[e] = ((keep >> e) & 1u) ? w[e] * p.dscale : 0.f;
       }
@@ -406,7 +406,7 @@
       }
       const int col = col_of(jp);
       if (p.drop_on) {
-        const uint32_t keep = dropout_keep8(rng, (uint64_t)((long)gm * N + col) >> 3, p.thresh);
+        const uint32_t keep = dropout_keep8(rng, (uint64_t)((long)gm * rng.row_mul * N + col) >> 3, p.thresh);
 #pragma unroll
         for (int e = 0; e < 8; ++e) w[e] = ((keep >> e) & 1u) ? w[e] * p.dscale : 0.f;
       }
diff --git a/vit-vs-raw-iq_amd/csrc/gemm_lnbwd.hip b/vit-vs-raw-iq_amd/csrc/gemm_lnbwd.hip
--- a/vit-vs-raw-iq_amd/csrc/gemm_lnbwd.hip
+++ b/vit-vs-raw-iq_amd/csrc/gemm_lnbwd.hip
@@ -243,7 +243,7 @@
         const long off = row * N + (v * LPR + lj) * 8;
         *reinterpret_cast<bf16x8*>(p.dZ + off) = pack8(o);
         if (p.drop_on) {
-          const uint32_t keep = dropout_keep8(rng, (uint64_t)off >> 3, p.thresh);
+          const uint32_t keep = dropout_keep8(rng, (uint64_t)(off + row * (long)(rng.row_mul - 1) * N) >> 3, p.thresh);
 #pragma unroll
           for (int e = 0; e < 8; ++e) o[e] = ((keep >> e) & 1u) ? o[e] * p.dscale : 0.f;
           *reinterpret_cast<bf16x8*>(p.dY + off) = pack8(o);
diff --git a/vit-vs-raw-iq_amd/csrc/layernorm.hip b/vit-vs-raw-iq_amd/csrc/layernorm.hip
--- a/vit-vs-raw-iq_amd/csrc/layernorm.hip
+++ b/vit-vs-raw-iq_amd/csrc/layernorm.hip
@@ -124,7 +124,7 @@
         if (MASK && (v * LPR + j) * 8 >= D) continue;
         *reinterpret_cast<bf16x8*>(dZ + off) = pack8(o);
         if (DROP) {
-          const uint32_t keep = dropout_keep8(rng, (uint64_t)off >> 3, thresh);
+          const uint32_t keep = dropout_keep8(rng, (uint64_t)(off + row * (long)(rng.row_mul - 1) * D) >> 3, thresh);
 #pragma unroll
           for (int e = 0; e < 8; ++e) o[e] = ((keep >> e) & 1u) ? o[e] * dscale : 0.f;
           *reinterpret_cast<bf16x8*>(dY + off) = pack8(o);
diff --git a/vit-vs-raw-iq_amd/csrc/misc.hip b/vit-vs-raw-iq_amd/csrc/misc.hip
--- a/vit-vs-raw-iq_amd/csrc/misc.hip
+++ b/vit-vs-raw-iq_amd/csrc/misc.hip
@@ -558,6 +558,7 @@
   IQ_PROF(IQ_FAM_MISC, stream);
   if (B <= 0) return IQ_OK;
   if (!cls || !pe || !x0 || (D % 8)) return IQ_ERR_ARG;
+  if (!dropout_rows_dense(drop)) return IQ_ERR_ARG;
   int on; IqRng r; uint32_t th; float sc;
   (void)dropout_unpack(drop, &on, &r, &th, &sc);
   const int n = B * (D / 8);
@@ -570,6 +571,7 @@
   IQ_PROF(IQ_FAM_MISC, stream);
   if (B <= 0) return IQ_OK;
   if (!dx0 || !demb || (D % 8) || (has_cls && !dcls)) return IQ_ERR_ARG;
+  if (!dropout_rows_dense(drop)) return IQ_ERR_ARG;
   int on; IqRng r; uint32_t th; float sc;
   (void)dropout_unpack(drop, &on, &r, &th, &sc);
   const size_t n = (size_t)B * tok * (D / 8);
@@ -703,6 +705,7 @@
                             hipStream_t st) {
   IQ_PROF(IQ_FAM_MISC, st);
   if (B <= 0) return IQ_OK;
+  if (!dropout_rows_dense(drop)) return IQ_ERR_ARG;
   int on; IqRng r; uint32_t th; float sc;
   (void)dropout_unpack(drop, &on, &r, &th, &sc);
   const size_t n = (size_t)B * tok * (D / 8);
diff --git a/vit-vs-raw-iq_amd/csrc/model.hip b/vit-vs-raw-iq_amd/csrc/model.hip
--- a/vit-vs-raw-iq_amd/csrc/model.hip
+++ b/vit-vs-raw-iq_amd/csrc/model.hip
@@ -15,6 +15,8 @@
                        int B, int S, int D, int K, int pool, hipStream_t st);
 int embed_bwd_gather_launch(const void* dx0, void* demb, int B, int S, int tok, int D, int has_cls, const iq_dropout_t* drop,
                             hipStream_t st);
+
+int attn_bwd_is_per_frame(int S, int H, int dh);
 
 namespace {
 
@@ -114,6 +116,17 @@
   float* rel;
   float* r[2];
 };
+
+__global__ void cls_scatter_kernel(const bf16* __restrict__ compact, bf16* __restrict__ dense, long n8, int S, int D8) {
+  for (long i = (long)blockIdx.x * blockDim.x + threadIdx.x; i < n8; i += (long)gridDim.x * blockDim.x) {
+    const long row = i / D8;
+    const int c = (int)(i - row * D8);
+    const long b = row / S;
+    bf16x8 v = {};
+    if (row - b * S == 0) v = reinterpret_cast<const bf16x8*>(compact)[b * D8 + c];
+    reinterpret_cast<bf16x8*>(dense)[i] = v;
+  }
+}
 
 __global__ void set_u32_kernel(uint32_t* p, uint32_t v, int bump) {
   if (threadIdx.x == 0 && blockIdx.x == 0) *p = bump ? *p + 1u : v;
@@ -149,12 +162,14 @@
   uint64_t last_seed = 0;
   bool last_tr = false;
   bool last_train_fwd = false;
+  bool last_cls = false;
+  bool last_cls_grad = false;
   const void* fwd_ws = nullptr;
   int fwd_batch = 0;
 
   iq_dropout_t bwd_site(uint32_t id, const uint32_t* step_dev, bool tr) const {
     iq_dropout_t d;
-    d.seed = last_seed; d.step = 0; d.site = id; d.p = tr ? c.drop_prob : 0.f; d.step_dev = step_dev;
+    d.seed = last_seed; d.step = 0; d.site = id; d.p = tr ? c.drop_prob : 0.f; d.row_mul = 0; d.step_dev = step_dev;
     return d;
   }
 
@@ -227,6 +242,7 @@
     g[3].N = (int)(3 * D); g[3].K = (int)D;
     mx(iq_wgrad_grouped_ws_bytes(g, 4, (int)M, 0));
     for (int k = 0; k < 4; ++k) mx(iq_wgrad_grouped_ws_bytes(g + k, 1, (int)M, 0));
+    mx(iq_wgrad_grouped_ws_bytes(g, 3, B, 0));
   }
   mx(iq_wgrad_ws_bytes((int)MT, (int)D, m->Ppad));
   w.wgrad_ws_bytes = wb;
@@ -256,6 +272,11 @@
   return tune >= 0 ? tune : M <= 32768 ? 3 : 2;
 }
 
+inline bool cls_route_supported(int D, int F) {
+  return iq_gemm_ln_supported(D, D) && iq_gemm_ln_supported(D, F) && iq_gemm_lnbwd_supported(D, F);
+}
+inline iq_dropout_t cls_rows(iq_dropout_t d, int S) { d.row_mul = (uint32_t)S; return d; }
+
 #define IQ_TRY(expr, what)                                                              \
   do {                                                                                  \
     int rc_ = (expr);                                                                   \
@@ -264,7 +285,7 @@
 
 iq_dropout_t site(const iq_model* m, uint64_t seed, const uint32_t* step_dev, uint32_t id, bool training) {
   iq_dropout_t d;
-  d.seed = seed; d.step = 0; d.site = id; d.p = training ? m->c.drop_prob : 0.f; d.step_dev = step_dev;
+  d.seed = seed; d.step = 0; d.site = id; d.p = training ? m->c.drop_prob : 0.f; d.row_mul = 0; d.step_dev = step_dev;
   return d;
 }
 
@@ -457,6 +478,10 @@
   const int D = c.d_model, F = c.ffn_hidden, S = m->S, H = c.n_head, B = batch;
   const int M = B * S, MT = B * m->tok;
   const bool tr = training != 0 && c.drop_prob > 0.f;
+  const bool logits_only = (training & IQ_FWD_LOGITS_ONLY) && logits && !enc_out && m->pool == 0 && m->has_cls && c.n_layers >= 1;
+  const bool cls_top = logits_only && !use_ffn_chain(M, S, D, F) && cls_route_supported(D, F);
+  m->last_cls = cls_top;
+  m->last_cls_grad = logits_only && !cls_top;
   uint32_t* step_dev = m->step_ctr ? m->step_ctr : (uint32_t*)(ws + w.step_ctr);
   m->last_tr = tr;
   m->last_train_fwd = true;
@@ -490,6 +515,22 @@
       IQ_TRY(iq_gemm_bf16_nt(x, D, m->sh(o.wqkv), D, ws + a.qkv, 3 * D, M, 3 * D, D, &e, stream), "qkv GEMM");
     }
     qkv_done = false;
+    if (cls_top && l == c.n_layers - 1) {
+      const int SD = S * D;
+      const iq_dropout_t c1 = cls_rows(site(m, seed, step_dev, 1 + 3 * l, tr), S);
+      const iq_dropout_t ch = cls_rows(site(m, seed, step_dev, 2 + 3 * l, tr), S);
+      const iq_dropout_t c2 = cls_rows(site(m, seed, step_dev, 3 + 3 * l, tr), S);
+      IQ_TRY(iq_attn_fwd_cls(ws + a.qkv, ws + a.att, (float*)(ws + a.lse), B, S, H, m->dh, stream), "attention fwd (CLS rows)");
+      IQ_TRY(iq_gemm_bf16_ln(ws + a.att, SD, m->sh(o.wo), D, P + o.bo, x, SD, &c1, P + o.g1, P + o.be1, 1e-12f, ws + a.z1, ws + a.x1,
+                             (float*)(ws + a.mean1), (float*)(ws + a.rstd1), B, D, D, stream), "out-proj GEMM + norm1 (CLS rows)");
+      memset(&e, 0, sizeof(e));
+      e.bias = P + o.b1; e.relu = 1; e.drop = ch;
+      IQ_TRY(iq_gemm_bf16_nt(ws + a.x1, D, m->sh(o.w1), D, ws + a.hid, F, B, F, D, &e, stream), "ffn1 GEMM (CLS rows)");
+      IQ_TRY(iq_gemm_bf16_ln(ws + a.hid, F, m->sh(o.w2), F, P + o.b2, ws + a.x1, D, &c2, P + o.g2, P + o.be2, 1e-12f, ws + a.z2,
+                             ws + a.x2, (float*)(ws + a.mean2), (float*)(ws + a.rstd2), B, D, F, stream), "ffn2 GEMM + norm2 (CLS rows)");
+      x = ws + a.x2;
+      continue;
+    }
     IQ_TRY(iq_attn_fwd(ws + a.qkv, ws + a.att, (float*)(ws + a.lse), B, S, H, m->dh, stream), "attention fwd");
     const iq_dropout_t dr1 = site(m, seed, step_dev, 1 + 3 * l, tr);
     const iq_dropout_t drh = site(m, seed, step_dev, 2 + 3 * l, tr);
@@ -538,7 +579,7 @@
   }
   if (logits) {
     IQ_TRY(iq_head_fwd(x, m->head_ln ? P + m->hln_g : nullptr, m->head_ln ? P + m->hln_b : nullptr, P + m->head_w,
-                       P + m->head_b, (float*)(ws + w.head_feat), (float*)(ws + w.head_stat), logits, B, S, D,
+                       P + m->head_b, (float*)(ws + w.head_feat), (float*)(ws + w.head_stat), logits, B, cls_top ? 1 : S, D,
                        c.num_classes, m->pool, stream), "head");
   }
   if (enc_out) bf16_to_f32_kernel<<<blocks_for((size_t)M * D / 8), 256, 0, st>>>((const bf16*)x, enc_out, (size_t)M * D / 8);
@@ -554,6 +595,9 @@
   if (m->fwd_batch != batch)
     return fail(m, IQ_ERR_ARG, std::string(what) + ": the last forward in this workspace had batch " + std::to_string(m->fwd_batch) +
                                    ", not " + std::to_string(batch));
+  if (m->last_cls)
+    return fail(m, IQ_ERR_ARG, std::string(what) + ": the last forward was a logits-only one (IQ_FWD_LOGITS_ONLY): its top layer "
+                                   "exists for the CLS rows only; run a dense forward first");
   *w = plan_ws(m, batch);
   if (ws_bytes < w->total) return fail(m, IQ_ERR_ARG, std::string(what) + ": workspace too small");
   return IQ_OK;
@@ -629,17 +673,22 @@
   float* G = m->grads;
   float* wws = (float*)(ws + w.wgrad_ws);
   const float dscale = tr ? dropout_scale(c.drop_prob) : 1.f;
+  const bool cls_top = m->last_cls;
+  if ((cls_top || m->last_cls_grad) && denc)
+    return fail(m, IQ_ERR_ARG, "backward: the last forward was a logits-only one (IQ_FWD_LOGITS_ONLY): no gradient can enter at "
+                               "the encoder output (denc); run a dense forward first");
+  const int Sh = cls_top ? 1 : S;
 
   if (stage_hi == Lr + 1) {
     if (!dlogits && !denc) return fail(m, IQ_ERR_ARG, "backward: dlogits or denc required at the head stage");
     if (dlogits && !pgrads) {
       IQ_TRY(head_bwd_dx_launch(dlogits, (const float*)(ws + w.head_feat), (const float*)(ws + w.head_stat),
-                                m->head_ln ? P + m->hln_g : nullptr, P + m->head_w, ws + w.gA, B, S, D, K, m->pool, st), "head bwd (dx)");
+                                m->head_ln ? P + m->hln_g : nullptr, P + m->head_w, ws + w.gA, B, Sh, D, K, m->pool, st), "head bwd (dx)");
     } else if (dlogits) {
       IQ_TRY(iq_head_bwd(dlogits, (const float*)(ws + w.head_feat), (const float*)(ws + w.head_stat),
                          m->head_ln ? P + m->hln_g : nullptr, m->head_ln ? P + m->hln_b : nullptr, P + m->head_w,
                          G + m->head_w, G + m->head_b, m->head_ln ? G + m->hln_g : nullptr,
-                         m->head_ln ? G + m->hln_b : nullptr, ws + w.gA, B, S, D, K, m->pool, accumulate, stream), "head bwd");
+                         m->head_ln ? G + m->hln_b : nullptr, ws + w.gA, B, Sh, D, K, m->pool, accumulate, stream), "head bwd");
     } else if (!accumulate && pgrads) {
       (void)hipMemsetAsync(G + m->head_begin, 0, (m->nparam - m->head_begin) * sizeof(float), st);
     }
@@ -657,6 +706,59 @@
     iq_epilogue_t e;
     float* lp2 = (float*)(ws + w.ln_part[0]);
     float* lp1 = (float*)(ws + w.ln_part[1]);
+    if (cls_top && l == Lr - 1) {
+      const int SD = S * D;
+      const iq_dropout_t c2 = cls_rows(m->bwd_site(3 + 3 * l, step_dev, tr), S);
+      const iq_dropout_t c1 = cls_rows(m->bwd_site(1 + 3 * l, step_dev, tr), S);
+      unsigned char* cZ1 = ws + w.gB;
+      IQ_TRY(iq_ln_bwd(ws + w.gA, ws + a.z2, (const float*)(ws + a.mean2), (const float*)(ws + a.rstd2), P + o.g2, gZ, gY, &c2,
+                       nullptr, nullptr, lp2, accumulate, B, D, stream), "norm2 bwd (CLS rows)");
+      const unsigned char* dO2 = tr ? gY : gZ;
+      memset(&e, 0, sizeof(e));
+      e.gate = ws + a.hid; e.ldg = F; e.gate_scale = dscale;
+      IQ_TRY(iq_gemm_bf16_nt(dO2, D, m->sht(o.t_w2), D, gH, F, B, F, D, &e, stream), "ffn2 dgrad (CLS rows)");
+      IQ_TRY(iq_gemm_bf16_lnbwd(gH, F, m->sht(o.t_w1), F, gZ, D, ws + a.z1, (const float*)(ws + a.mean1), (const float*)(ws + a.rstd1),
+                                P + o.g1, &c1, cZ1, gY1, lp1, B, D, F, stream), "ffn1 dgrad + norm1 bwd (CLS rows)");
+      const unsigned char* dAo = tr ? gY1 : cZ1;
+      IQ_TRY(iq_gemm_bf16_nt(dAo, D, m->sht(o.t_wo), D, ws + w.gAtt, SD, B, D, D, nullptr, stream), "out-proj dgrad (CLS rows)");
+      IQ_TRY(iq_attn_bwd_cls(ws + a.qkv, ws + a.att, ws + w.gAtt, (const float*)(ws + a.lse), gQKV, B, S, H, m->dh, stream),
+             "attention bwd (CLS rows)");
+      {
+        IQ_PROF(IQ_FAM_MISC, st);
+        const long n8 = (long)M * D / 8;
+        cls_scatter_kernel<<<blocks_for((size_t)n8), 256, 0, st>>>((const bf16*)cZ1, (bf16*)gZ1, n8, S, D / 8);
+        IQ_PROF_K(2.0 * ((double)M * D + (double)B * D), 0.0, "cls_scatter_kernel");
+      }
+      if (pgrads) {
+        const iq_wgrad_problem_t wc[3] = {
+            {dO2, D, ws + a.hid, F, G + o.w2, G + o.b2, D, F},
+            {gH, F, ws + a.x1, D, G + o.w1, G + o.b1, F, D},
+            {dAo, D, ws + a.att, SD, G + o.wo, G + o.bo, D, D}};
+        const iq_wgrad_problem_t wq = {gQKV, 3 * D, xin, D, G + o.wqkv, G + o.bqkv, 3 * D, D};
+        const int rows2 = iq_ln_bwd_partial_rows(B, D), rows1 = iq_gemm_lnbwd_partial_rows(B);
+        const iq_reduce_seg_t lnseg[4] = {{lp2, rows2, 2L * D, G + o.g2, D}, {lp2 + D, rows2, 2L * D, G + o.be2, D},
+                                          {lp1, rows1, 2L * D, G + o.g1, D}, {lp1 + D, rows1, 2L * D, G + o.be1, D}};
+        IQ_TRY(iq_gemm_bf16_wgrad_grouped(wc, 3, B, wws, w.wgrad_ws_bytes, accumulate, 0, lnseg, 4, stream),
+               "layer weight gradients (CLS rows)");
+        IQ_TRY(iq_gemm_bf16_wgrad_grouped(&wq, 1, M, wws, w.wgrad_ws_bytes, accumulate, 0, nullptr, 0, stream), "q,k,v weight gradient");
+      }
+      const bool chain_below = fuse1 && m->last_train_fwd && use_ffn_chain(M, S, D, F) && use_chain_pre(M) >= 3;
+      deferred = l > 0 && fuse2 && chain_below && sidx - 1 >= stage_lo;
+      if (deferred) continue;
+      if (l > 0 && fuse2) {
+        const LayerOff& ob = m->L[l - 1];
+        const WsPlan::L& ab = w.layers[l - 1];
+        const iq_dropout_t dr2b = m->bwd_site(3 + 3 * (l - 1), step_dev, tr);
+        IQ_TRY(iq_gemm_bf16_lnbwd(gQKV, 3 * D, m->sht(o.t_wqkv), 3 * D, gZ1, D, ws + ab.z2, (const float*)(ws + ab.mean2),
+                                  (const float*)(ws + ab.rstd2), P + ob.g2, &dr2b, gZ, gY, lp2, M, D, 3 * D, stream),
+               "qkv dgrad + norm2 bwd of the layer below");
+      } else {
+        memset(&e, 0, sizeof(e));
+        e.residual = gZ1; e.ldr = D;
+        IQ_TRY(iq_gemm_bf16_nt(gQKV, 3 * D, m->sht(o.t_wqkv), 3 * D, ws + w.gA, D, M, D, 3 * D, &e, stream), "qkv dgrad");
+      }
+      continue;
+    }
     const bool norm2_here = l == Lr - 1 || !fuse2;
     if (norm2_here) {
       const iq_dropout_t dr2 = m->bwd_site(3 + 3 * l, step_dev, tr);
@@ -717,6 +819,10 @@
       }
       if (l == 0) break;
     }
+    if (m->last_cls_grad && l == Lr - 1 && !attn_bwd_is_per_frame(S, H, m->dh))
+      IQ_TRY(iq_attn_bwd_cls(ws + a.qkv, ws + a.att, ws + w.gAtt, (const float*)(ws + a.lse), gQKV, B, S, H, m->dh, stream),
+             "attention bwd (dO in the CLS rows only)");
+    else
     IQ_TRY(iq_attn_bwd(ws + a.qkv, ws + a.att, ws + w.gAtt, (const float*)(ws + a.lse), gQKV, B, S, H, m->dh, stream), "attention bwd");
     if (pgrads) IQ_TRY(iq_gemm_bf16_wgrad_grouped(wg, 4, M, wws, w.wgrad_ws_bytes, accumulate, 0, lnseg, 4, stream), "layer weight gradients");
     deferred = l > 0 && fuse2 && chain && post && use_chain_pre(M) >= 3 && sidx - 1 >= stage_lo;
diff --git a/vit-vs-raw-iq_amd/trainer.py b/vit-vs-raw-iq_amd/trainer.py
--- a/vit-vs-raw-iq_amd/trainer.py
+++ b/vit-vs-raw-iq_amd/trainer.py
@@ -159,8 +159,9 @@
 
         def fwd_and_first_bucket():
             st = N.stream_handle()
-            N.check(L.iq_model_forward(plan.h, x.data_ptr(), B, ws.data_ptr(), ws.numel(), 1, plan.seed, step_arg, None,
-                                       self._logits.data_ptr(), st), "iq_model_forward", plan.h)
+            N.check(L.iq_model_forward(plan.h, x.data_ptr(), B, ws.data_ptr(), ws.numel(),
+                                       N.FWD_TRAIN | N.FWD_LOGITS_ONLY,
+                                       plan.seed, step_arg, None, self._logits.data_ptr(), st), "iq_model_forward", plan.h)
             N.check(L.iq_ce_fwd_bwd(self._logits.data_ptr(), y.data_ptr(), B, plan.cfg.num_classes, self.smoothing,
                                     float(B), self.loss_sum.data_ptr(), self.n_correct.data_ptr(),
                                     self._dlogits.data_ptr(), st), "iq_ce_fwd_bwd")
```
